# Glaciohound/Chimera-ST

Measured on AMD Instinct MI355X. Metric: train utterances/sec, MuST-C EN-DE s2t_transformer_m, 1/2/4/8 MI355X, higher is better.
Workload: dtype bf16

## Files before the change

chimera-st_amd/csrc/attention.hip:

```cpp
#include "cst_common.h"
#include <stdlib.h>
#include <type_traits>

namespace {

constexpr int NW = 4;
constexpr int QB = 32;
constexpr int KT = 64;

struct AttnParams {
  int64_t B, H, Tq, Tk;
  const void *Q, *K, *V; void* O;
  int64_t q_sb, q_sh, q_st, k_sb, k_sh, k_st, v_sb, v_sh, v_st, o_sb, o_sh, o_st;
  float* lse;
  const uint8_t* kpm; int64_t kpm_stride;
  int causal;
  float scale;
  const void* dO; int64_t do_sb, do_sh, do_st;
  void *dQ, *dK, *dV;
  int64_t dq_sb, dq_sh, dq_st, dk_sb, dk_sh, dk_st, dv_sb, dv_sh, dv_st;
  float* delta;
  uint32_t drop_thr, drop_key; float drop_scale;
  const int32_t* kv_len;
  uint8_t* q_flags;
  const int32_t* seq_off;
  const unsigned long long* kpm_bits; int64_t kpm_bits_stride;
};

struct SeqView { int64_t row0; int tq, tk; };
__device__ __forceinline__ SeqView seq_view(const AttnParams& p, int64_t b) {
  SeqView v;
  if (p.seq_off) {
    v.row0 = p.seq_off[b];
    v.tq = p.seq_off[b + 1] - p.seq_off[b];
    v.tk = p.kv_len ? (p.kv_len[b] < v.tq ? p.kv_len[b] : v.tq) : v.tq;
    if (v.tk < 0) v.tk = 0;
  } else {
    v.row0 = 0;
    v.tq = (int)p.Tq;
    v.tk = (int)p.Tk;
  }
  return v;
}

__device__ __forceinline__ int live_query_end(const AttnParams& p, int64_t b, int64_t h, int* sh, int tid, int tq) {
  const int nqt = (int)((p.Tq + 63) / 64);
  if (!p.q_flags) return tq;
  if (tid < 64) {
    const uint8_t* f = p.q_flags + (b * p.H + h) * nqt;
    int last = -1;
    for (int base = 0; base < nqt; base += 64) {
      const int idx = base + tid;
      const unsigned long long m = __ballot(idx < nqt && f[idx < nqt ? idx : 0] != 0);
      if (m) last = base + 63 - __clzll(m);
    }
    if (tid == 0) *sh = (last + 1) * 64;
  }
  __syncthreads();
  const int e = *sh;
  return e < tq ? e : tq;
}

__device__ __forceinline__ int slot_row(int t, int j, int hi) { return 16 * t + (j & 3) + 8 * (j >> 2) + 4 * hi; }

template <typename T, int D>
struct TileRegs {
  static constexpr int VEC = DT<T>::VEC, VPR = D / VEC, NV = (KT * VPR + NW * 64 - 1) / (NW * 64);
  u32x4 r[NV];
  __device__ __forceinline__ void fetch(const T* g, int64_t st, int nrows, int tid) {
#pragma unroll
    for (int i = 0; i < NV; ++i) {
      const int v = tid + NW * 64 * i;
      int row = v / VPR;
      row = row < nrows ? row : nrows - 1;
      if (v < KT * VPR) r[i] = *reinterpret_cast<const u32x4*>(g + (int64_t)row * st + (v % VPR) * VEC);
    }
  }
  __device__ __forceinline__ void stage(T* lds, int tid) const {
    constexpr int LD = D + VEC;
#pragma unroll
    for (int i = 0; i < NV; ++i) {
      const int v = tid + NW * 64 * i;
      if (v < KT * VPR) *reinterpret_cast<u32x4*>(lds + (v / VPR) * LD + (v % VPR) * VEC) = r[i];
    }
  }
};

template <typename T, int D>
__device__ __forceinline__ void load_row_frags(Frag<T> (&f)[D / 16], const T* g, int64_t st, int row, int nrows, int lane) {
  const int lk = 8 * (lane >> 5);
#pragma unroll
  for (int kk = 0; kk < D / 16; ++kk) {
    if (row < nrows) frag_load_contig(f[kk], g + (int64_t)row * st + kk * 16 + lk);
    else {
      float z[8] = {0, 0, 0, 0, 0, 0, 0, 0};
      frag_from_f32(f[kk], z);
    }
  }
}

template <typename T>
__device__ __forceinline__ void store_dcol(T* g, const f32x16& acc, int d0, int lane, float mul) {
  const int hi = lane >> 5;
#pragma unroll
  for (int gq = 0; gq < 4; ++gq) {
    T* p = g + d0 + 8 * gq + 4 * hi;
#pragma unroll
    for (int e = 0; e < 4; ++e) DT<T>::st(p + e, acc[gq * 4 + e] * mul);
  }
}

template <typename T, int D, bool DROP>
__global__ __launch_bounds__(NW * 64, (sizeof(T) == 2 ? 3 : 2)) void attn_fwd_kernel(AttnParams p) {
  constexpr int VEC = DT<T>::VEC, LD = D + VEC, TILE = KT * LD;
  extern __shared__ __attribute__((aligned(16))) char smem_raw[];
  T* smem = reinterpret_cast<T*>(smem_raw);
  unsigned long long* sMask = reinterpret_cast<unsigned long long*>(smem + 4 * TILE);
  const int tid = threadIdx.x, lane = tid & 63, wave = tid >> 6, hi = lane >> 5;
  const int64_t b = blockIdx.z, h = blockIdx.y;
  const int q_blk0 = blockIdx.x * (NW * QB);
  const int q = q_blk0 + wave * QB + (lane & 31);
  const SeqView sv = seq_view(p, b);
  if (q_blk0 >= sv.tq) return;
  const T* Qg = (const T*)p.Q + (p.seq_off ? sv.row0 * p.q_st : b * p.q_sb) + h * p.q_sh;
  const T* Kg = (const T*)p.K + (p.seq_off ? sv.row0 * p.k_st : b * p.k_sb) + h * p.k_sh;
  const T* Vg = (const T*)p.V + (p.seq_off ? sv.row0 * p.v_st : b * p.v_sb) + h * p.v_sh;
  const int cshift = sv.tk - sv.tq;
  const float c2 = p.scale * 1.4426950408889634f;
  const uint32_t dkey2 = cst_drop_key2(p.drop_key);
  const int thr_s = (int)p.drop_thr - 32768;
  const uint32_t rho = (uint32_t)((b * p.H + h) * p.Tq + q);
  cst_i32x4 bsig = {0, 0, 0, 0};
  if (DROP) bsig = cst_asig_row_frag(p.drop_key, dkey2, rho, hi);

  Frag<T> fq[D / 16];
  load_row_frags<T, D>(fq, Qg, p.q_st, q, sv.tq, lane);

  f32x16 o[D / 32];
#pragma unroll
  for (int dt = 0; dt < D / 32; ++dt)
#pragma unroll
    for (int r = 0; r < 16; ++r) o[dt][r] = 0.0f;
  float m_run = -1.0e30f, l_run = 0.0f;

  int64_t kend = sv.tk;
  if (!p.seq_off && p.kv_len && p.kv_len[b] < kend) kend = p.kv_len[b] > 0 ? p.kv_len[b] : 0;
  if (p.causal) {
    const int64_t last = (int64_t)q_blk0 + NW * QB - 1 + cshift + 1;
    if (last < kend) kend = last;
  }
  TileRegs<T, D> rk, rv;
  uint8_t rmask = 0;
  auto prefetch = [&](int64_t j0) {
    const int nk = (int)((sv.tk - j0 < KT) ? (sv.tk - j0) : KT);
    rk.fetch(Kg + j0 * p.k_st, p.k_st, nk, tid);
    rv.fetch(Vg + j0 * p.v_st, p.v_st, nk, tid);
    if (tid < KT) rmask = (tid >= nk) ? 1 : (p.kpm ? p.kpm[b * p.kpm_stride + j0 + tid] : 0);
  };
  auto stage = [&](int st) {
    rk.stage(smem + st * 2 * TILE, tid);
    rv.stage(smem + st * 2 * TILE + TILE, tid);
    if (wave == 0) {
      const unsigned long long bits = __ballot(rmask != 0);
      if (lane == 0) sMask[st] = bits;
    }
  };
  if (kend > 0) { prefetch(0); stage(0); }
  __syncthreads();
  int cur = 0;
  const int qlo = q_blk0 + wave * QB;
  for (int64_t j0 = 0; j0 < kend; j0 += KT) {
    const bool more = j0 + KT < kend;
    if (more) prefetch(j0 + KT);
    const T* sK = smem + cur * 2 * TILE;
    const T* sV = sK + TILE;
    const unsigned long long mb = sMask[cur];

    f32x16 s[2];
#pragma unroll
// ... 305 lines not shown

  f32x16 dk[D / 32], dv[D / 32];
#pragma unroll
  for (int dt = 0; dt < D / 32; ++dt)
#pragma unroll
    for (int r = 0; r < 16; ++r) { dk[dt][r] = 0.0f; dv[dt][r] = 0.0f; }

  int64_t qstart = 0;
  if (p.causal) {
    qstart = (int64_t)k_blk0 - cshift;
    if (qstart < 0) qstart = 0;
    qstart = (qstart / KT) * KT;
  }
  TileRegs<T, D> rq, rdo;
  float rl = -INFINITY, rd = 0.0f;
  auto prefetch = [&](int64_t i0) {
    const int nq = (int)((sv.tq - i0 < KT) ? (sv.tq - i0) : KT);
    rq.fetch(Qg + i0 * p.q_st, p.q_st, nq, tid);
    rdo.fetch(dOg + i0 * p.do_st, p.do_st, nq, tid);
    if (tid < KT) {
      const float l = tid < nq ? p.lse[(b * p.H + h) * p.Tq + i0 + tid] : -INFINITY;
      rl = l == -INFINITY ? INFINITY : l * 1.4426950408889634f;
      rd = tid < nq ? p.delta[(b * p.H + h) * p.Tq + i0 + tid] : 0.0f;
    }
  };
  auto stage = [&](int st) {
    rq.stage(smem + st * 2 * TILE, tid);
    rdo.stage(smem + st * 2 * TILE + TILE, tid);
    if (tid < KT) { sStat[st * 2 * KT + tid] = rl; sStat[st * 2 * KT + KT + tid] = rd; }
  };
  const int64_t qlim = live_query_end(p, b, h, reinterpret_cast<int*>(sStat + 4 * KT), tid, sv.tq);
  if (qstart < qlim) { prefetch(qstart); stage(0); }
  __syncthreads();
  int cur = 0;
  for (int64_t i0 = qstart; i0 < qlim; i0 += KT) {
    const bool more = i0 + KT < qlim;
    if (more) prefetch(i0 + KT);
    const T* sQ = smem + cur * 2 * TILE;
    const T* sdO = sQ + TILE;
    const float* sL = sStat + cur * 2 * KT;
    const float* sD = sL + KT;
#pragma unroll
    for (int qs = 0; qs < 2; ++qs) {
      f32x16 s, dp;
#pragma unroll
      for (int r = 0; r < 16; ++r) { s[r] = 0.0f; dp[r] = 0.0f; }
#pragma unroll
      for (int kk = 0; kk < D / 16; ++kk) {
        Frag<T> fqr, fdor;
        frag_load_contig(fqr, sQ + (qs * 32 + (lane & 31)) * LD + kk * 16 + 8 * hi);
        frag_load_contig(fdor, sdO + (qs * 32 + (lane & 31)) * LD + kk * 16 + 8 * hi);
        mma16(s, fqr, fk[kk]);
        mma16(dp, fdor, fv[kk]);
      }
      f32x16 pr;
      const bool diag = p.causal && (k_blk0 + wave * QB + QB - 1 > (int)i0 + qs * 32 + cshift);
      uint32_t keepbits = 0;
      if (DROP) {
        const cst_i32x16 dm = cst_asig_block(cst_asig_row_frag(p.drop_key, dkey2, rho0 + (uint32_t)((int)i0 + qs * 32 + (lane & 31)), hi), ksig);
#pragma unroll
        for (int r = 0; r < 16; ++r) keepbits |= (cst_adrop_keep(dm[r], thr_s) ? 1u : 0u) << r;
      }
#pragma unroll
      for (int r = 0; r < 16; ++r) {
        const int qr = qs * 32 + acc_row(r, lane);
        const float l = sL[qr];
        float e = __builtin_amdgcn_exp2f(fmaf(s[r], c2, -l));
        if (diag) e = (key > (int)i0 + qr + cshift) ? 0.0f : e;
        float dpr = dp[r];
        if (DROP) {
          const bool keep = (keepbits >> r) & 1u;
          dpr = keep ? dpr * p.drop_scale : 0.0f;
          pr[r] = keep ? e * p.drop_scale : 0.0f;
        } else {
          pr[r] = e;
        }
        s[r] = e * (dpr - sD[qr]);
      }
#pragma unroll
      for (int t = 0; t < 2; ++t) {
        Frag<T> fp, fds;
        float x[8], y[8];
#pragma unroll
        for (int j = 0; j < 8; ++j) { x[j] = pr[8 * t + j]; y[j] = s[8 * t + j]; }
        frag_from_f32(fp, x);
        frag_from_f32(fds, y);
#pragma unroll
        for (int dt = 0; dt < D / 32; ++dt) {
          Frag<T> fdot, fqt;
          frag_load_tr(fdot, sdO, LD, dt * 32, qs * 32 + 16 * t + 4 * hi, qs * 32 + 16 * t + 4 * hi + 8, lane);
          frag_load_tr(fqt, sQ, LD, dt * 32, qs * 32 + 16 * t + 4 * hi, qs * 32 + 16 * t + 4 * hi + 8, lane);
          mma16(dv[dt], fdot, fp);
          mma16(dk[dt], fqt, fds);
        }
      }
    }
    if (more) stage(cur ^ 1);
    __syncthreads();
    cur ^= 1;
  }
  if (key_masked) {
#pragma unroll
    for (int dt = 0; dt < D / 32; ++dt)
#pragma unroll
      for (int r = 0; r < 16; ++r) { dk[dt][r] = 0.0f; dv[dt][r] = 0.0f; }
  }
  if (key < krows) {
    T* gk = dKb + (int64_t)key * p.dk_st;
    T* gv = dVb + (int64_t)key * p.dv_st;
#pragma unroll
    for (int dt = 0; dt < D / 32; ++dt) {
      store_dcol<T>(gk, dk[dt], dt * 32, lane, p.scale);
      store_dcol<T>(gv, dv[dt], dt * 32, lane, 1.0f);
    }
  }
}

#include "attention_fast.inc"

int fill_params(const cst_attn_desc* d, AttnParams& p, bool bwd) {
  CST_REQUIRE(d, "cst_attn: null descriptor");
  CST_REQUIRE(d->dtype == CST_F32 || d->dtype == CST_BF16, "cst_attn: bad dtype %d", d->dtype);
  CST_REQUIRE(d->D == 32 || d->D == 64, "cst_attn: head dim %lld not in {32,64}", (long long)d->D);
  CST_REQUIRE(d->B > 0 && d->H > 0 && d->Tq > 0 && d->Tk > 0, "cst_attn: empty problem");
  CST_REQUIRE(d->Q && d->K && d->V && d->O && d->lse, "cst_attn: null tensor");
  CST_REQUIRE(d->H < 65536 && d->B < 65536, "cst_attn: B/H too large for the grid");
  const int vec = d->dtype == CST_BF16 ? 8 : 4;
  const int64_t strides[] = {d->q_sb, d->q_sh, d->q_st, d->k_sb, d->k_sh, d->k_st, d->v_sb, d->v_sh, d->v_st};
  for (int64_t s : strides) CST_REQUIRE(s % vec == 0, "cst_attn: strides must be multiples of %d elements", vec);
  CST_REQUIRE(((uintptr_t)d->Q % 16 == 0) && ((uintptr_t)d->K % 16 == 0) && ((uintptr_t)d->V % 16 == 0), "cst_attn: Q/K/V must be 16-byte aligned");
  p.B = d->B; p.H = d->H; p.Tq = d->Tq; p.Tk = d->Tk;
  p.Q = d->Q; p.K = d->K; p.V = d->V; p.O = d->O;
  p.q_sb = d->q_sb; p.q_sh = d->q_sh; p.q_st = d->q_st;
  p.k_sb = d->k_sb; p.k_sh = d->k_sh; p.k_st = d->k_st;
  p.v_sb = d->v_sb; p.v_sh = d->v_sh; p.v_st = d->v_st;
  p.o_sb = d->o_sb; p.o_sh = d->o_sh; p.o_st = d->o_st;
  p.lse = d->lse; p.kpm = d->key_padding_mask; p.kpm_stride = d->kpm_stride;
  p.causal = d->causal; p.scale = d->scale;
  CST_REQUIRE(d->drop_p >= 0.0f && d->drop_p < 1.0f, "cst_attn: drop_p must be in [0, 1)");
  CST_REQUIRE(d->drop_p == 0.0f || (double)d->B * d->H * d->Tq < 4294967296.0, "cst_attn: dropout row space exceeds 2^32 rows");
  p.drop_thr = d->drop_p > 0.0f ? cst_drop_thr16(d->drop_p) : 0u;
  p.drop_key = d->drop_key;
  p.drop_scale = d->drop_p > 0.0f ? 1.0f / (1.0f - d->drop_p) : 1.0f;
  p.dO = d->dO; p.do_sb = d->do_sb; p.do_sh = d->do_sh; p.do_st = d->do_st;
  p.dQ = d->dQ; p.dK = d->dK; p.dV = d->dV;
  p.dq_sb = d->dq_sb; p.dq_sh = d->dq_sh; p.dq_st = d->dq_st;
  p.dk_sb = d->dk_sb; p.dk_sh = d->dk_sh; p.dk_st = d->dk_st;
  p.dv_sb = d->dv_sb; p.dv_sh = d->dv_sh; p.dv_st = d->dv_st;
  p.delta = d->delta;
  p.kv_len = d->kv_len;
  p.seq_off = d->seq_offsets;
  p.kpm_bits = (const unsigned long long*)d->kpm_bits;
  p.kpm_bits_stride = (d->Tk + 63) / 64;
  if (p.seq_off) {
    CST_REQUIRE(d->Tq == d->Tk && d->key_padding_mask == nullptr, "cst_attn: packed sequences are self-attention (Tq == Tk = longest segment) without a key padding mask (kv_len gives the keys per sequence)");
    CST_REQUIRE(d->q_st == d->k_st && d->q_st == d->v_st, "cst_attn: packed Q/K/V must share one row stride");
  }
  p.q_flags = bwd ? d->q_flags : nullptr;
  if (bwd) {
    CST_REQUIRE(d->dO && d->dQ && d->dK && d->dV && d->delta, "cst_attn_bwd: null gradient tensor");
    CST_REQUIRE(d->do_sb % vec == 0 && d->do_sh % vec == 0 && d->do_st % vec == 0 && d->o_st % vec == 0 && d->o_sb % vec == 0 && d->o_sh % vec == 0,
                "cst_attn_bwd: dO/O strides must be multiples of %d", vec);
    CST_REQUIRE(((uintptr_t)d->dO % 16 == 0) && ((uintptr_t)d->O % 16 == 0), "cst_attn_bwd: dO/O must be 16-byte aligned");
  }
  return CST_OK;
}

template <typename T, int D>
constexpr size_t attn_lds_bytes() {
  return 4 * (size_t)KT * (D + DT<T>::VEC) * sizeof(T) + 4 * KT * sizeof(float) + 16;
}
void attn_set_lds(const void* fn) {
  (void)hipFuncSetAttribute(fn, hipFuncAttributeMaxDynamicSharedMemorySize, 96 * 1024);
}

double attn_flops(const cst_attn_desc* d, double gemms) {
  double pairs = (double)d->Tq * (double)d->Tk;
  if (d->causal) pairs *= 0.5;
  return gemms * 2.0 * pairs * (double)d->D * (double)d->B * (double)d->H;
}

bool attn_fast_ok(const cst_attn_desc* d) {
  const bool off = getenv("CST_ATTN_GENERIC") != nullptr;
  return !off && d->dtype == CST_BF16 && d->D == 64 && !d->causal && (d->key_padding_mask == nullptr || d->kpm_bits != nullptr) &&
         d->Tk <= 65536 && (int64_t)d->Tk * d->k_st < (1ll << 29) && (int64_t)d->Tq * d->q_st < (1ll << 29) && (int64_t)d->Tk * d->v_st < (1ll << 29) &&
         d->o_st % 8 == 0 && d->o_sh % 8 == 0 && d->o_sb % 8 == 0 && (uintptr_t)d->O % 16 == 0;
}
bool attn_fast_bwd_ok(const cst_attn_desc* d) {
  const int64_t st[] = {d->dq_sb, d->dq_sh, d->dq_st, d->dk_sb, d->dk_sh, d->dk_st, d->dv_sb, d->dv_sh, d->dv_st};
  for (int64_t x : st) if (x % 8) return false;
  return attn_fast_ok(d) && d->bwd_ws != nullptr && (uintptr_t)d->dQ % 16 == 0 && (uintptr_t)d->dK % 16 == 0 && (uintptr_t)d->dV % 16 == 0 &&
         (uintptr_t)d->bwd_ws % 16 == 0 && (int64_t)d->Tq * d->do_st < (1ll << 29);
}

}

extern "C" int cst_attn_fwd(const cst_attn_desc* d, cst_stream stream) {
  AttnParams p;
  int rc = fill_params(d, p, false);
  if (rc != CST_OK) return rc;
  hipStream_t s = (hipStream_t)stream;
  if (attn_fast_ok(d)) {
    CstProfScope prof(CST_K_ATTN_FWD, s, attn_flops(d, 2.0), 0.0);
    const unsigned nblk = fa_grid(d->Tq, d->B, d->H);
    const size_t lds = FA_NSLOT * FA_SLOT + 8 * (size_t)cst_ceil_div(d->Tk, 64) + (p.drop_thr ? 4096 : 0);
    if (p.drop_thr) hipLaunchKernelGGL((fa_fwd_kernel<true>), dim3(nblk), dim3(256), lds, s, p);
    else hipLaunchKernelGGL((fa_fwd_kernel<false>), dim3(nblk), dim3(256), lds, s, p);
    return cst_check_launch("cst_attn_fwd");
  }
  dim3 grid((unsigned)cst_ceil_div(d->Tq, NW * QB), (unsigned)d->H, (unsigned)d->B);
  CstProfScope prof(CST_K_ATTN_FWD, s, attn_flops(d, 2.0), 0.0);
#define CST_FWD1(T, DD, DR) do { const size_t lds = attn_lds_bytes<T, DD>(); attn_set_lds(reinterpret_cast<const void*>(&attn_fwd_kernel<T, DD, DR>)); \
    hipLaunchKernelGGL((attn_fwd_kernel<T, DD, DR>), grid, dim3(NW * 64), lds, s, p); } while (0)
#define CST_FWD(T, DD) do { if (p.drop_thr) CST_FWD1(T, DD, true); else CST_FWD1(T, DD, false); } while (0)
  if (d->dtype == CST_BF16) { if (d->D == 64) CST_FWD(bf16_t, 64); else CST_FWD(bf16_t, 32); }
  else { if (d->D == 64) CST_FWD(float, 64); else CST_FWD(float, 32); }
#undef CST_FWD
#undef CST_FWD1
  return cst_check_launch("cst_attn_fwd");
}

int cst_fa_dec_cross(const void* q, const void* kx, const void* vx, const uint8_t* kpm, void* out, const int32_t* step, int64_t max_len,
                     int64_t bsz, int64_t beam, int64_t H, int64_t S, float scale, const void* Wg, const float* sg, const float* sb, float eps,
                     int64_t K, int64_t ldx, hipStream_t s) {
  if (Wg) {
    FdProj pj = {(const bf16_t*)Wg, sg, sb, eps, (int)K, (long long)ldx};
    return fa_dec_cross_launch(q, kx, vx, kpm, out, step, max_len, bsz, beam, H, S, scale, &pj, s);
  }
  return fa_dec_cross_launch(q, kx, vx, kpm, out, step, max_len, bsz, beam, H, S, scale, nullptr, s);
}

extern "C" int64_t cst_attn_bwd_workspace(const cst_attn_desc* d) {
  if (!d) return 0;
  return (int64_t)d->B * d->H * cst_ceil_div(d->Tq, 64) * 64 * (int64_t)(2 * sizeof(float) + 32);
}

extern "C" int cst_attn_bwd(const cst_attn_desc* d, cst_stream stream) {
  AttnParams p;
  int rc = fill_params(d, p, true);
  if (rc != CST_OK) return rc;
  hipStream_t s = (hipStream_t)stream;
  CstProfScope prof(CST_K_ATTN_BWD, s, attn_flops(d, 5.0), 0.0);
  if (attn_fast_bwd_ok(d)) {
    const int64_t Tq64 = cst_ceil_div(d->Tq, 64) * 64;
    float* ws = (float*)d->bwd_ws;
    static const bool delta_pass = getenv("CST_ATTN_DELTA_PASS") != nullptr;
    if (delta_pass) hipLaunchKernelGGL(fa_delta_kernel, dim3((unsigned)(Tq64 / 64), (unsigned)d->H, (unsigned)d->B), dim3(64), 0, s, p, ws, Tq64);
    const unsigned nq = fa_grid(d->Tq, d->B, d->H), nk = fa_grid(d->Tk, d->B, d->H);
    const size_t lds_q = FA_NSLOT * FA_SLOT + 8 * (size_t)cst_ceil_div(d->Tk, 64) + (p.drop_thr ? 4096 : 0) + 16, lds_k = FA_NSLOT * (FA_SLOT + FA_STATS);
    if (p.drop_thr) {
      hipLaunchKernelGGL((fa_dq_kernel<true>), dim3(nq), dim3(256), lds_q, s, p, ws, Tq64);
      hipLaunchKernelGGL((fa_dkv_kernel<true>), dim3(nk), dim3(256), lds_k, s, p, (const float*)ws, Tq64);
    } else {
      hipLaunchKernelGGL((fa_dq_kernel<false>), dim3(nq), dim3(256), lds_q, s, p, ws, Tq64);
      hipLaunchKernelGGL((fa_dkv_kernel<false>), dim3(nk), dim3(256), lds_k, s, p, (const float*)ws, Tq64);
    }
    return cst_check_launch("cst_attn_bwd");
  }
  dim3 gq((unsigned)cst_ceil_div(d->Tq, NW * QB), (unsigned)d->H, (unsigned)d->B);
  dim3 gk((unsigned)cst_ceil_div(d->Tk, NW * QB), (unsigned)d->H, (unsigned)d->B);
#define CST_BWD1(T, DD, DR)                                                                                \
  do {                                                                                                     \
    hipLaunchKernelGGL((attn_delta_kernel<T, DD>), dim3((unsigned)cst_ceil_div(d->Tq, 64), (unsigned)d->H, (unsigned)d->B), dim3(64), 0, s, p); \
    const size_t lds = attn_lds_bytes<T, DD>();                                                              \
    attn_set_lds(reinterpret_cast<const void*>(&attn_bwd_dq_kernel<T, DD, DR>));                             \
    attn_set_lds(reinterpret_cast<const void*>(&attn_bwd_dkv_kernel<T, DD, DR>));                            \
    hipLaunchKernelGGL((attn_bwd_dq_kernel<T, DD, DR>), gq, dim3(NW * 64), lds, s, p);                      \
    hipLaunchKernelGGL((attn_bwd_dkv_kernel<T, DD, DR>), gk, dim3(NW * 64), lds, s, p);                     \
  } while (0)
#define CST_BWD(T, DD) do { if (p.drop_thr) CST_BWD1(T, DD, true); else CST_BWD1(T, DD, false); } while (0)
  if (d->dtype == CST_BF16) { if (d->D == 64) CST_BWD(bf16_t, 64); else CST_BWD(bf16_t, 32); }
  else { if (d->D == 64) CST_BWD(float, 64); else CST_BWD(float, 32); }
#undef CST_BWD
#undef CST_BWD1
  return cst_check_launch("cst_attn_bwd");
}
```

chimera-st_amd/csrc/attention_fast.inc:

```

typedef int fa_i32x4 __attribute__((ext_vector_type(4)));
constexpr int FA_IMG = 64 * 128;
constexpr int FA_SLOT = 2 * FA_IMG;
constexpr int FA_NSLOT = 3;
constexpr float FA_THR = 8.0f;

__device__ __forceinline__ int fa_sw(int r) {
  const int s = (r >> 1) & 7;
  return s ^ ((s & 1) << 2);
}
__device__ __forceinline__ fa_i32x4 fa_rsrc(const void* base, uint32_t bytes) {
  const unsigned long long a = (unsigned long long)base;
  fa_i32x4 r;
  r[0] = __builtin_amdgcn_readfirstlane((int)(unsigned)a);
  r[1] = __builtin_amdgcn_readfirstlane((int)(unsigned)(a >> 32));
  r[2] = __builtin_amdgcn_readfirstlane((int)bytes);
  r[3] = 0x00020000;
  return r;
}
__device__ __forceinline__ void fa_dma16(const fa_i32x4& rs, unsigned lds, unsigned voff) {
  unsigned keep;
  asm volatile("s_mov_b32 %0, m0\n\ts_mov_b32 m0, %1\n\ts_nop 0\n\tbuffer_load_dwordx4 %2, %3, 0 offen lds\n\ts_mov_b32 m0, %0"
               : "=&s"(keep) : "s"(lds), "v"(voff), "s"(rs) : "memory");
}
__device__ __forceinline__ void fa_dma4(const fa_i32x4& rs, unsigned lds, unsigned voff) {
  unsigned keep;
  asm volatile("s_mov_b32 %0, m0\n\ts_mov_b32 m0, %1\n\ts_nop 0\n\tbuffer_load_dword %2, %3, 0 offen lds\n\ts_mov_b32 m0, %0"
               : "=&s"(keep) : "s"(lds), "v"(voff), "s"(rs) : "memory");
}
__device__ __forceinline__ void fa_dma_tile4(const fa_i32x4& rsA, const fa_i32x4& rsB, unsigned lds, unsigned a0, unsigned a1, unsigned b0, unsigned b1) {
  unsigned keep;
  asm volatile("s_mov_b32 %0, m0\n\ts_mov_b32 m0, %1\n\ts_nop 0\n\tbuffer_load_dwordx4 %2, %6, 0 offen lds\n\t"
               "s_add_i32 m0, %1, 0x400\n\ts_nop 0\n\tbuffer_load_dwordx4 %3, %6, 0 offen lds\n\t"
               "s_add_i32 m0, %1, 0x2000\n\ts_nop 0\n\tbuffer_load_dwordx4 %4, %7, 0 offen lds\n\t"
               "s_add_i32 m0, %1, 0x2400\n\ts_nop 0\n\tbuffer_load_dwordx4 %5, %7, 0 offen lds\n\ts_mov_b32 m0, %0"
               : "=&s"(keep) : "s"(lds), "v"(a0), "v"(a1), "v"(b0), "v"(b1), "s"(rsA), "s"(rsB) : "memory");
}
template <int N> __device__ __forceinline__ void fa_wait_vm() { asm volatile("s_waitcnt vmcnt(%0)" ::"n"(N) : "memory"); }

__device__ __forceinline__ void fa_dma_lanes(unsigned (&v)[2], int64_t st, int wave, int lane) {
#pragma unroll
  for (int i = 0; i < 2; ++i) {
    const int row = 8 * (2 * wave + i) + (lane >> 3);
    v[i] = (unsigned)(row * (int)st * 2 + ((((lane & 7) ^ fa_sw(row))) << 4));
  }
}
struct FaLanes {
  unsigned row[4];
  unsigned ta[2];
  unsigned tb[2];
};
__device__ __forceinline__ FaLanes fa_lanes(int lane) {
  FaLanes L;
  const int hi = lane >> 5, lrow = lane & 31, swl = fa_sw(lrow);
#pragma unroll
  for (int kk = 0; kk < 4; ++kk) L.row[kk] = (unsigned)(lrow * 128 + (((2 * kk + hi) ^ swl) << 4));
  const int s = lane & 15, r0 = 4 * hi + (s >> 2), cc = 2 * ((lane >> 4) & 1) + ((s & 3) >> 1), cb = 8 * (s & 1);
#pragma unroll
  for (int dt = 0; dt < 2; ++dt) {
    L.ta[dt] = (unsigned)(r0 * 128 + (((4 * dt + cc) ^ fa_sw(r0)) << 4) + cb);
    L.tb[dt] = (unsigned)((r0 + 8) * 128 + (((4 * dt + cc) ^ fa_sw(r0 + 8)) << 4) + cb);
  }
  return L;
}
__device__ __forceinline__ bf16x8 fa_ld_row(const char* img, unsigned off) { return *reinterpret_cast<const bf16x8*>(img + off); }
__device__ __forceinline__ bf16x8 fa_ld_tr(const char* img, unsigned oa, unsigned ob) {
  const v4s_t x = __builtin_amdgcn_ds_read_tr16_b64_v4i16((v4s_t __attribute__((address_space(3)))*)(img + oa));
  const v4s_t y = __builtin_amdgcn_ds_read_tr16_b64_v4i16((v4s_t __attribute__((address_space(3)))*)(img + ob));
  u16x8 t;
  t[0] = (unsigned short)x[0]; t[1] = (unsigned short)x[1]; t[2] = (unsigned short)x[2]; t[3] = (unsigned short)x[3];
  t[4] = (unsigned short)y[0]; t[5] = (unsigned short)y[1]; t[6] = (unsigned short)y[2]; t[7] = (unsigned short)y[3];
  return __builtin_bit_cast(bf16x8, t);
}
typedef short fa_s16x2 __attribute__((ext_vector_type(2)));
typedef float fa_f32x2 __attribute__((ext_vector_type(2)));
typedef __bf16 fa_bf16x2 __attribute__((ext_vector_type(2)));
__device__ __forceinline__ unsigned fa_pack2(float lo, float hi) {
  const fa_f32x2 v = {lo, hi};
  return __builtin_bit_cast(unsigned, __builtin_convertvector(v, fa_bf16x2));
}
__device__ __forceinline__ fa_s16x2 fa_thrm1(uint32_t thr16) {
  const short t = (short)((int)thr16 - 32768 - 1);
  fa_s16x2 v = {t, t};
  return v;
}
__device__ __forceinline__ unsigned fa_keep_pair(unsigned packed, int d0, int d1, fa_s16x2 thrm1) {
  fa_s16x2 h = __builtin_bit_cast(fa_s16x2, __builtin_amdgcn_perm((unsigned)d1, (unsigned)d0, 0x05040100u));
  h = h << 2;
  fa_s16x2 t = __builtin_elementwise_sub_sat(thrm1, h);
  t = t >> 15;
  return packed & __builtin_bit_cast(unsigned, t);
}
template <bool KEYS>
__device__ __forceinline__ void fa_stage_sigs(char* dst, uint32_t key, uint32_t key2, uint32_t row0, int tid) {
  const uint32_t r = row0 + (uint32_t)(tid >> 2);
  const int w = 2 * (tid & 3);
  uint2 v;
  v.x = KEYS ? cst_asig_key(key, key2, r, w) : cst_asig_row(key, key2, r, w);
  v.y = KEYS ? cst_asig_key(key, key2, r, w + 1) : cst_asig_row(key, key2, r, w + 1);
  *reinterpret_cast<uint2*>(dst + (tid >> 2) * 32 + (tid & 3) * 8) = v;
}
__device__ __forceinline__ cst_i32x16 fa_mask_block(const char* sigs, int blk, int lane, const cst_i32x4& own) {
  const cst_i32x4 a = *reinterpret_cast<const cst_i32x4*>(sigs + (blk * 32 + (lane & 31)) * 32 + 16 * (lane >> 5));
  return cst_asig_block(a, own);
}
#define FA_MFMA(a, b, c) __builtin_amdgcn_mfma_f32_32x32x16_bf16(a, b, c, 0, 0, 0)

__device__ __forceinline__ float fa_other_half(float x) {
  const unsigned u = __float_as_uint(x);
  const auto r = __builtin_amdgcn_permlane32_swap(u, u, false, false);
  return __uint_as_float((threadIdx.x & 32) ? r[0] : r[1]);
}
__device__ __forceinline__ void fa_row_frags(bf16x8 (&f)[4], const bf16_t* g, int64_t st, int row, int nrows, int hi, float mul) {
  const int rc = row < nrows ? row : nrows - 1;
  const float m = row < nrows ? mul : 0.0f;
  u32x4 raw[4];
#pragma unroll
  for (int kk = 0; kk < 4; ++kk) raw[kk] = *reinterpret_cast<const u32x4*>(g + (int64_t)rc * st + kk * 16 + 8 * hi);
#pragma unroll
  for (int kk = 0; kk < 4; ++kk) {
    u32x4 w;
#pragma unroll
    for (int i = 0; i < 4; ++i) w[i] = fa_pack2(__uint_as_float(raw[kk][i] << 16) * m, __uint_as_float(raw[kk][i] & 0xffff0000u) * m);
    f[kk] = __builtin_bit_cast(bf16x8, w);
  }
}
template <typename T> __device__ __forceinline__ const T* fa_uniform(const T* p) {
  const unsigned long long a = (unsigned long long)p;
  const unsigned lo = (unsigned)__builtin_amdgcn_readfirstlane((int)(unsigned)a), hi = (unsigned)__builtin_amdgcn_readfirstlane((int)(unsigned)(a >> 32));
  return (const T*)(((unsigned long long)hi << 32) | lo);
}
__device__ __forceinline__ unsigned long long fa_tile_bits(const unsigned long long* kb_lds, int j, int kend) {
  if (kb_lds) {
    const unsigned long long v = kb_lds[j];
    const unsigned lo = (unsigned)__builtin_amdgcn_readfirstlane((int)(unsigned)v), hi = (unsigned)__builtin_amdgcn_readfirstlane((int)(unsigned)(v >> 32));
    return ((unsigned long long)hi << 32) | lo;
  }
  const int left = kend - 64 * j;
  return left >= 64 ? 0ull : (~0ull << left);
}
__device__ __forceinline__ void fa_store_row(bf16_t* rowp, const f32x16 (&acc)[2], float mul, int hi) {
#pragma unroll
  for (int dt = 0; dt < 2; ++dt)
#pragma unroll
    for (int gp = 0; gp < 2; ++gp) {
      unsigned a[2], c[2];
#pragma unroll
      for (int e = 0; e < 2; ++e) {
        a[e] = fa_pack2(acc[dt][8 * gp + 2 * e] * mul, acc[dt][8 * gp + 2 * e + 1] * mul);
        c[e] = fa_pack2(acc[dt][8 * gp + 4 + 2 * e] * mul, acc[dt][8 * gp + 4 + 2 * e + 1] * mul);
      }
      const auto r0 = __builtin_amdgcn_permlane32_swap(a[0], c[0], false, false);
      const auto r1 = __builtin_amdgcn_permlane32_swap(a[1], c[1], false, false);
      u32x4 v = {r0[0], r1[0], r0[1], r1[1]};
      *reinterpret_cast<u32x4*>(rowp + dt * 32 + 16 * gp + 8 * hi) = v;
    }
}

__device__ __forceinline__ bool fa_block_coords(const AttnParams& p, int nxb, int& xb, int64_t& h, int64_t& b) {
  const unsigned id = blockIdx.x, xcd = id & 7, k = id >> 3;
  const unsigned g = (k / (unsigned)nxb) * 8 + xcd;
  xb = __builtin_amdgcn_readfirstlane((int)(k % (unsigned)nxb));
  h = __builtin_amdgcn_readfirstlane((int)(g % (unsigned)p.H));
  b = __builtin_amdgcn_readfirstlane((int)(g / (unsigned)p.H));
  return g < (unsigned)(p.B * p.H);
}
inline unsigned fa_grid(int64_t rows, int64_t B, int64_t H) { return (unsigned)(8 * cst_ceil_div(rows, 128) * cst_ceil_div(B * H, 8)); }

#ifdef CST_TRACE
#define FA_STAMP(i) do { if (tr && tid == 0) { tr[2 * (i)] = (long long)__builtin_readcyclecounter(); tr[2 * (i) + 1] = (long long)__builtin_amdgcn_s_memrealtime(); } } while (0)
#else
#define FA_STAMP(i) do { } while (0)
#endif

template <bool DROP>
__global__ __launch_bounds__(256, 3) void fa_fwd_kernel(AttnParams p) {
  extern __shared__ __attribute__((aligned(16))) char smem_raw[];
  const int tid = threadIdx.x, lane = tid & 63, hi = lane >> 5;
  const int wave = __builtin_amdgcn_readfirstlane(tid >> 6);
#ifdef CST_TRACE
  long long* tr = p.delta ? reinterpret_cast<long long*>(p.delta) + (size_t)blockIdx.x * 16 : nullptr;
#endif
  FA_STAMP(0);
  int xb; int64_t b, h;
  if (!fa_block_coords(p, (int)((p.Tq + 127) / 128), xb, h, b)) return;
  const int q_blk0 = xb * 128;
  const SeqView sv = seq_view(p, b);
  if (q_blk0 >= sv.tq) return;
  const int q = q_blk0 + wave * 32 + (lane & 31);
  const bf16_t* Qg = (const bf16_t*)p.Q + (p.seq_off ? sv.row0 * p.q_st : b * p.q_sb) + h * p.q_sh;
  const bf16_t* Kg = (const bf16_t*)p.K + (p.seq_off ? sv.row0 * p.k_st : b * p.k_sb) + h * p.k_sh;
  const bf16_t* Vg = (const bf16_t*)p.V + (p.seq_off ? sv.row0 * p.v_st : b * p.v_sb) + h * p.v_sh;
  int kend = sv.tk;
  if (!p.seq_off && p.kv_len && p.kv_len[b] < kend) kend = p.kv_len[b] > 0 ? p.kv_len[b] : 0;
  const int ntiles = (kend + 63) >> 6;
  const int ntmax = (int)((p.Tk + 63) >> 6);
  unsigned long long* kbits = p.kpm_bits ? reinterpret_cast<unsigned long long*>(smem_raw + FA_NSLOT * FA_SLOT) : nullptr;
  char* const sigs = smem_raw + FA_NSLOT * FA_SLOT + 8 * ntmax;
  const unsigned lds0 = (unsigned)(uintptr_t)(__attribute__((address_space(3))) char*)smem_raw;
  const fa_i32x4 rsK = fa_rsrc(Kg, kend > 0 ? (uint32_t)((kend - 1) * p.k_st * 2 + 128) : 0u);
  const fa_i32x4 rsV = fa_rsrc(Vg, kend > 0 ? (uint32_t)((kend - 1) * p.v_st * 2 + 128) : 0u);
  unsigned vk[2], vv[2];
  fa_dma_lanes(vk, p.k_st, wave, lane);
  fa_dma_lanes(vv, p.v_st, wave, lane);
  const unsigned stepK = (unsigned)(64 * p.k_st * 2), stepV = (unsigned)(64 * p.v_st * 2);
  auto dma_tile = [&](int j, int slot) {
    fa_dma_tile4(rsK, rsV, lds0 + slot * FA_SLOT + wave * 2048, vk[0] + (unsigned)j * stepK, vk[1] + (unsigned)j * stepK,
                 vv[0] + (unsigned)j * stepV, vv[1] + (unsigned)j * stepV);
  };
  if (ntiles > 0) dma_tile(0, 0);
  if (ntiles > 1) dma_tile(1, 1);

  const float c2 = p.scale * 1.4426950408889634f;
  bf16x8 fq[4];
  fa_row_frags(fq, Qg, p.q_st, q, sv.tq, hi, c2);
  const uint32_t dkey2 = cst_drop_key2(p.drop_key);
  cst_i32x4 bsig = {0, 0, 0, 0};
  if (DROP) {
    bsig = cst_asig_row_frag(p.drop_key, dkey2, (uint32_t)((b * p.H + h) * p.Tq + q), hi);
    fa_stage_sigs<true>(sigs, p.drop_key, dkey2, 0u, tid);
  }
  if (kbits) for (int j = tid; j < ntiles; j += 256) kbits[j] = p.kpm_bits[b * p.kpm_bits_stride + j];
  const FaLanes L = fa_lanes(lane);
  const fa_s16x2 thrm1 = fa_thrm1(p.drop_thr);

  f32x16 o[2], negm;
#pragma unroll
  for (int r = 0; r < 16; ++r) { o[0][r] = 0.0f; o[1][r] = 0.0f; negm[r] = 0.0f; }
  float l_run = 0.0f, raise_at = -INFINITY;

  FA_STAMP(1);
  fa_wait_vm<0>();
  __syncthreads();
  FA_STAMP(2);

  auto tile = [&](int j, auto slot_c) {
    constexpr int SLOT = decltype(slot_c)::value;
    const bool ahead = j + 2 < ntiles;
    if (ahead) dma_tile(j + 2, (SLOT + 2) % FA_NSLOT);
    const char* sK = smem_raw + SLOT * FA_SLOT;
    const char* sV = sK + FA_IMG;
    const unsigned long long mb = fa_tile_bits(kbits, j, kend);
    f32x16 s[2];
    if (__builtin_expect(mb != 0ull, 0)) {
      const unsigned long long mbl = mb >> (4 * hi);
#pragma unroll
      for (int ks = 0; ks < 2; ++ks) {
        f32x16 cm;
#pragma unroll
        for (int r = 0; r < 16; ++r) cm[r] = ((mbl >> (ks * 32 + (r & 3) + 8 * (r >> 2))) & 1ull) ? -INFINITY : negm[r];
        s[ks] = FA_MFMA(fa_ld_row(sK, L.row[0] + ks * 4096), fq[0], cm);
#pragma unroll
        for (int kk = 1; kk < 4; ++kk) s[ks] = FA_MFMA(fa_ld_row(sK, L.row[kk] + ks * 4096), fq[kk], s[ks]);
      }
    } else {
#pragma unroll
      for (int ks = 0; ks < 2; ++ks) {
        s[ks] = FA_MFMA(fa_ld_row(sK, L.row[0] + ks * 4096), fq[0], negm);
#pragma unroll
        for (int kk = 1; kk < 4; ++kk) s[ks] = FA_MFMA(fa_ld_row(sK, L.row[kk] + ks * 4096), fq[kk], s[ks]);
      }
    }
    float mt = s[0][0];
#pragma unroll
    for (int ks = 0; ks < 2; ++ks)
#pragma unroll
      for (int r = 0; r < 16; ++r) mt = fmaxf(mt, s[ks][r]);
    mt = fmaxf(mt, fa_other_half(mt));
    if (__builtin_expect(__any(mt > raise_at), 0)) {
      const bool need = mt > raise_at;
      const bool first = raise_at < 0.0f;
      const float dm = need ? ceilf(mt) : 0.0f;
      const float alpha = first ? 1.0f : __builtin_amdgcn_exp2f(-dm);
#pragma unroll
      for (int r = 0; r < 16; ++r) { o[0][r] *= alpha; o[1][r] *= alpha; negm[r] -= dm; s[0][r] -= dm; s[1][r] -= dm; }
      l_run *= alpha;
      raise_at = need ? FA_THR : raise_at;
    }
    fa_f32x2 l01 = {0.0f, 0.0f};
#pragma unroll
    for (int ks = 0; ks < 2; ++ks)
#pragma unroll
      for (int r = 0; r < 16; r += 2) {
        s[ks][r] = __builtin_amdgcn_exp2f(s[ks][r]);
        s[ks][r + 1] = __builtin_amdgcn_exp2f(s[ks][r + 1]);
        const fa_f32x2 pr = {s[ks][r], s[ks][r + 1]};
        l01 = l01 + pr;
      }
    l_run += l01[0] + l01[1];
    unsigned pk[2][8];
#pragma unroll
    for (int ks = 0; ks < 2; ++ks)
#pragma unroll
      for (int i = 0; i < 8; ++i) pk[ks][i] = fa_pack2(s[ks][2 * i], s[ks][2 * i + 1]);
    if (DROP) {
      if (j + 1 < ntiles) fa_stage_sigs<true>(sigs + ((j + 1) & 1) * 2048, p.drop_key, dkey2, (uint32_t)(64 * (j + 1)), tid);
#pragma unroll
      for (int ks = 0; ks < 2; ++ks) {
        const cst_i32x16 dm = fa_mask_block(sigs + (j & 1) * 2048, ks, lane, bsig);
#pragma unroll
        for (int i = 0; i < 8; ++i) pk[ks][i] = fa_keep_pair(pk[ks][i], dm[2 * i], dm[2 * i + 1], thrm1);
      }
    }
#pragma unroll
    for (int ks = 0; ks < 2; ++ks)
#pragma unroll
      for (int t = 0; t < 2; ++t) {
        const u32x4 fpw = {pk[ks][4 * t], pk[ks][4 * t + 1], pk[ks][4 * t + 2], pk[ks][4 * t + 3]};
        const bf16x8 fp = __builtin_bit_cast(bf16x8, fpw);
#pragma unroll
        for (int dt = 0; dt < 2; ++dt)
          o[dt] = FA_MFMA(fa_ld_tr(sV, L.ta[dt] + ks * 4096 + t * 2048, L.tb[dt] + ks * 4096 + t * 2048), fp, o[dt]);
      }
    if (ahead) fa_wait_vm<4>(); else fa_wait_vm<0>();
    if (DROP) __syncthreads();
    else __builtin_amdgcn_s_barrier();
  };
  for (int j = 0; j < ntiles; j += 3) {
    tile(j, std::integral_constant<int, 0>{});
    if (j + 1 < ntiles) tile(j + 1, std::integral_constant<int, 1>{});
    if (j + 2 < ntiles) tile(j + 2, std::integral_constant<int, 2>{});
  }
  FA_STAMP(3);
  const float l_tot = l_run + fa_other_half(l_run);
  if (q < sv.tq) {
    const float inv = l_tot > 0.0f ? p.drop_scale / l_tot : 0.0f;
    bf16_t* Og = (bf16_t*)p.O + (p.seq_off ? sv.row0 * p.o_st : b * p.o_sb) + h * p.o_sh + (int64_t)q * p.o_st;
    fa_store_row(Og, o, inv, hi);
    if (hi == 0) p.lse[(b * p.H + h) * p.Tq + q] = l_tot > 0.0f ? (__log2f(l_tot) - negm[0]) * 0.6931471805599453f : -INFINITY;
  }
#ifdef CST_TRACE
  FA_STAMP(4);
  if (tr && tid == 0) { tr[10] = (long long)__builtin_amdgcn_s_getreg(4 | (0 << 6) | (31 << 11)); tr[11] = ntiles; }
#endif
}

__global__ __launch_bounds__(64) void fa_delta_kernel(AttnParams p, float* ws, int64_t Tq64) {
  const int64_t b = blockIdx.z, h = blockIdx.y;
  const int qt = blockIdx.x, lane = threadIdx.x;
  const int rl = lane >> 3, c8 = (lane & 7) * 8;
  bool nz = false;
  const SeqView sv = seq_view(p, b);
  const bf16_t* obase = (const bf16_t*)p.O + (p.seq_off ? sv.row0 * p.o_st : b * p.o_sb) + h * p.o_sh + c8;
  const bf16_t* gbase = (const bf16_t*)p.dO + (p.seq_off ? sv.row0 * p.do_st : b * p.do_sb) + h * p.do_sh + c8;
  float* w0 = ws + ((b * p.H + h) * 2) * Tq64;
  const float inv_ds = 1.0f / p.drop_scale;
#pragma unroll
  for (int it = 0; it < 8; ++it) {
    const int64_t q = (int64_t)qt * 64 + it * 8 + rl;
    float acc = 0.0f;
    if (q < sv.tq) {
      float a[8], c[8];
      load8(obase + q * p.o_st, a);
      load8(gbase + q * p.do_st, c);
#pragma unroll
      for (int e = 0; e < 8; ++e) { acc += a[e] * c[e]; nz = nz || c[e] != 0.0f; }
    }
    acc += __shfl_xor(acc, 1, 64);
    acc += __shfl_xor(acc, 2, 64);
    acc += __shfl_xor(acc, 4, 64);
    if ((lane & 7) == 0) {
      float nl = -INFINITY;
      if (q < sv.tq) {
        const float l = p.lse[(b * p.H + h) * p.Tq + q];
        nl = l == -INFINITY ? -INFINITY : -l * 1.4426950408889634f;
      }
      w0[q] = nl;
      w0[Tq64 + q] = q < sv.tq ? -acc * inv_ds : 0.0f;
    }
  }
  const unsigned long long m = __ballot(nz);
  if (p.q_flags && lane == 0) p.q_flags[(b * p.H + h) * ((p.Tq + 63) / 64) + qt] = m != 0ull ? 1 : 0;
}

__device__ __forceinline__ f32x16 fa_masked_c(const f32x16& c, unsigned long long mbl, int ks) {
  f32x16 cm;
#pragma unroll
  for (int r = 0; r < 16; ++r) cm[r] = ((mbl >> (ks * 32 + (r & 3) + 8 * (r >> 2))) & 1ull) ? -INFINITY : c[r];
  return cm;
}

template <bool DROP>
__global__ __launch_bounds__(256, 2) void fa_dq_kernel(AttnParams p, float* ws, int64_t Tq64) {
  extern __shared__ __attribute__((aligned(16))) char smem_raw[];
  const int tid = threadIdx.x, lane = tid & 63, hi = lane >> 5;
  const int wave = __builtin_amdgcn_readfirstlane(tid >> 6);
  int xb; int64_t b, h;
  if (!fa_block_coords(p, (int)((p.Tq + 127) / 128), xb, h, b)) return;
  const int q_blk0 = xb * 128;
  const SeqView sv = seq_view(p, b);
  const int nqt = (int)((p.Tq + 63) / 64);
  uint8_t* const qfl = p.q_flags ? p.q_flags + (b * p.H + h) * nqt + 2 * xb : nullptr;
  if (q_blk0 >= sv.tq) {
    if (qfl && tid < 2 && 2 * xb + tid < nqt) qfl[tid] = 0;
    return;
  }
  const int q = q_blk0 + wave * 32 + (lane & 31);
  const bf16_t* Qg = (const bf16_t*)p.Q + (p.seq_off ? sv.row0 * p.q_st : b * p.q_sb) + h * p.q_sh;
  const bf16_t* Kg = (const bf16_t*)p.K + (p.seq_off ? sv.row0 * p.k_st : b * p.k_sb) + h * p.k_sh;
  const bf16_t* Vg = (const bf16_t*)p.V + (p.seq_off ? sv.row0 * p.v_st : b * p.v_sb) + h * p.v_sh;
  const bf16_t* dOg = (const bf16_t*)p.dO + (p.seq_off ? sv.row0 * p.do_st : b * p.do_sb) + h * p.do_sh;
  const bf16_t* Og = (const bf16_t*)p.O + (p.seq_off ? sv.row0 * p.o_st : b * p.o_sb) + h * p.o_sh;
  bf16_t* const dQb = (bf16_t*)p.dQ + (p.seq_off ? sv.row0 * p.dq_st : b * p.dq_sb) + h * p.dq_sh;
  int kend = sv.tk;
  if (!p.seq_off && p.kv_len && p.kv_len[b] < kend) kend = p.kv_len[b] > 0 ? p.kv_len[b] : 0;
  const int ntiles = (kend + 63) >> 6;
  const int ntmax = (int)((p.Tk + 63) >> 6);
  unsigned long long* kbits = p.kpm_bits ? reinterpret_cast<unsigned long long*>(smem_raw + FA_NSLOT * FA_SLOT) : nullptr;
  char* const sigs = smem_raw + FA_NSLOT * FA_SLOT + 8 * ntmax;
  int* const sh_nz = reinterpret_cast<int*>(smem_raw + FA_NSLOT * FA_SLOT + 8 * ntmax + (DROP ? 4096 : 0));
  const unsigned lds0 = (unsigned)(uintptr_t)(__attribute__((address_space(3))) char*)smem_raw;
  const fa_i32x4 rsK = fa_rsrc(Kg, kend > 0 ? (uint32_t)((kend - 1) * p.k_st * 2 + 128) : 0u);
  const fa_i32x4 rsV = fa_rsrc(Vg, kend > 0 ? (uint32_t)((kend - 1) * p.v_st * 2 + 128) : 0u);
  unsigned vk[2], vv[2];
  fa_dma_lanes(vk, p.k_st, wave, lane);
  fa_dma_lanes(vv, p.v_st, wave, lane);
  const unsigned stepK = (unsigned)(64 * p.k_st * 2), stepV = (unsigned)(64 * p.v_st * 2);
  auto dma_tile = [&](int j, int slot) {
    fa_dma_tile4(rsK, rsV, lds0 + slot * FA_SLOT + wave * 2048, vk[0] + (unsigned)j * stepK, vk[1] + (unsigned)j * stepK,
                 vv[0] + (unsigned)j * stepV, vv[1] + (unsigned)j * stepV);
  };
  if (ntiles > 0) dma_tile(0, 0);
  if (ntiles > 1) dma_tile(1, 1);

  const float c2 = p.scale * 1.4426950408889634f;
  bf16x8 fq[4], fdo[4];
  fa_row_frags(fq, Qg, p.q_st, q, sv.tq, hi, c2);
  fa_row_frags(fdo, dOg, p.do_st, q, sv.tq, hi, 1.0f);
  float ndv, nl = -INFINITY;
  bool nzrow = false;
  {
    float acc = 0.0f;
    const int rc = q < sv.tq ? q : sv.tq - 1;
#pragma unroll
    for (int kk = 0; kk < 4; ++kk) {
      const u32x4 ro = *reinterpret_cast<const u32x4*>(Og + (int64_t)rc * p.o_st + kk * 16 + 8 * hi);
      const u32x4 rg = __builtin_bit_cast(u32x4, fdo[kk]);
#pragma unroll
      for (int i = 0; i < 4; ++i) {
        acc += __uint_as_float(ro[i] << 16) * __uint_as_float(rg[i] << 16);
        acc += __uint_as_float(ro[i] & 0xffff0000u) * __uint_as_float(rg[i] & 0xffff0000u);
        nzrow = nzrow || (rg[i] & 0x7fff7fffu) != 0u;
      }
    }
    acc += __shfl_xor(acc, 32, 64);
    if (q < sv.tq) {
      const float l = p.lse[(b * p.H + h) * p.Tq + q];
      nl = l == -INFINITY ? -INFINITY : -l * 1.4426950408889634f;
    }
    ndv = q < sv.tq ? -acc * (1.0f / p.drop_scale) : 0.0f;
    if (hi == 0 && q < Tq64) {
      float* w0 = ws + ((b * p.H + h) * 2) * Tq64;
      w0[q] = nl;
      w0[Tq64 + q] = ndv;
    }
    const unsigned long long m = __ballot(nzrow);
    if (lane == 0) sh_nz[wave] = m != 0ull ? 1 : 0;
  }
  f32x16 nl2, nd, dq[2];
#pragma unroll
  for (int r = 0; r < 16; ++r) { nl2[r] = nl; nd[r] = ndv; dq[0][r] = 0.0f; dq[1][r] = 0.0f; }
  const uint32_t dkey2 = cst_drop_key2(p.drop_key);
  const int thr_s = (int)p.drop_thr - 32768;
  cst_i32x4 bsig = {0, 0, 0, 0};
  if (DROP) {
    bsig = cst_asig_row_frag(p.drop_key, dkey2, (uint32_t)((b * p.H + h) * p.Tq + q), hi);
    fa_stage_sigs<true>(sigs, p.drop_key, dkey2, 0u, tid);
    if (q < Tq64) {
      cst_i32x4* sg = reinterpret_cast<cst_i32x4*>(reinterpret_cast<char*>(ws + (size_t)p.B * p.H * 2 * Tq64) + ((size_t)(b * p.H + h) * Tq64 + q) * 32 + 16 * hi);
      *sg = bsig;
    }
  }
  if (kbits) for (int j = tid; j < ntiles; j += 256) kbits[j] = p.kpm_bits[b * p.kpm_bits_stride + j];
  const FaLanes L = fa_lanes(lane);
  fa_wait_vm<0>();
  __syncthreads();
  {
    const int nz01 = sh_nz[0] | sh_nz[1], nz23 = sh_nz[2] | sh_nz[3];
    if (qfl && tid == 0) {
      qfl[0] = (uint8_t)nz01;
      if (2 * xb + 1 < nqt) qfl[1] = (uint8_t)nz23;
    }
    if (!(nz01 | nz23)) {
      if (q < sv.tq) {
        f32x16 z[2];
#pragma unroll
        for (int r = 0; r < 16; ++r) { z[0][r] = 0.0f; z[1][r] = 0.0f; }
        fa_store_row(dQb + (int64_t)q * p.dq_st, z, 1.0f, hi);
      }
      return;
    }
  }

  auto tile = [&](int j, auto slot_c) {
    constexpr int SLOT = decltype(slot_c)::value;
    const bool ahead = j + 2 < ntiles;
    if (ahead) dma_tile(j + 2, (SLOT + 2) % FA_NSLOT);
    const char* sK = smem_raw + SLOT * FA_SLOT;
    const char* sV = sK + FA_IMG;
    const unsigned long long mb = fa_tile_bits(kbits, j, kend);
    const unsigned long long mbl = mb >> (4 * hi);
    if (DROP && j + 1 < ntiles) fa_stage_sigs<true>(sigs + ((j + 1) & 1) * 2048, p.drop_key, dkey2, (uint32_t)(64 * (j + 1)), tid);
#pragma unroll
    for (int ks = 0; ks < 2; ++ks) {
      f32x16 s, dp;
      if (__builtin_expect(mb != 0ull, 0)) s = FA_MFMA(fa_ld_row(sK, L.row[0] + ks * 4096), fq[0], fa_masked_c(nl2, mbl, ks));
      else s = FA_MFMA(fa_ld_row(sK, L.row[0] + ks * 4096), fq[0], nl2);
      dp = FA_MFMA(fa_ld_row(sV, L.row[0] + ks * 4096), fdo[0], nd);
#pragma unroll
      for (int kk = 1; kk < 4; ++kk) {
        s = FA_MFMA(fa_ld_row(sK, L.row[kk] + ks * 4096), fq[kk], s);
        dp = FA_MFMA(fa_ld_row(sV, L.row[kk] + ks * 4096), fdo[kk], dp);
      }
      if (DROP) {
        const cst_i32x16 dm = fa_mask_block(sigs + (j & 1) * 2048, ks, lane, bsig);
#pragma unroll
        for (int r = 0; r < 16; ++r) dp[r] = cst_adrop_keep(dm[r], thr_s) ? dp[r] : ndv;
      }
#pragma unroll
      for (int r = 0; r < 16; ++r) s[r] = __builtin_amdgcn_exp2f(s[r]) * dp[r];
#pragma unroll
      for (int t = 0; t < 2; ++t) {
        const u32x4 fw = {fa_pack2(s[8 * t], s[8 * t + 1]), fa_pack2(s[8 * t + 2], s[8 * t + 3]), fa_pack2(s[8 * t + 4], s[8 * t + 5]), fa_pack2(s[8 * t + 6], s[8 * t + 7])};
        const bf16x8 fds = __builtin_bit_cast(bf16x8, fw);
#pragma unroll
        for (int dt = 0; dt < 2; ++dt)
          dq[dt] = FA_MFMA(fa_ld_tr(sK, L.ta[dt] + ks * 4096 + t * 2048, L.tb[dt] + ks * 4096 + t * 2048), fds, dq[dt]);
      }
    }
    if (ahead) fa_wait_vm<4>(); else fa_wait_vm<0>();
    if (DROP) __syncthreads();
    else __builtin_amdgcn_s_barrier();
  };
  for (int j = 0; j < ntiles; j += 3) {
    tile(j, std::integral_constant<int, 0>{});
    if (j + 1 < ntiles) tile(j + 1, std::integral_constant<int, 1>{});
    if (j + 2 < ntiles) tile(j + 2, std::integral_constant<int, 2>{});
  }
  if (q < sv.tq) fa_store_row(dQb + (int64_t)q * p.dq_st, dq, p.scale * p.drop_scale, hi);
}

constexpr int FA_STATS = 2 * 256 + 2048;

template <bool DROP>
__global__ __launch_bounds__(256, 2) void fa_dkv_kernel(AttnParams p, const float* ws, int64_t Tq64) {
  extern __shared__ __attribute__((aligned(16))) char smem_raw[];
  constexpr int SLOTB = FA_SLOT + FA_STATS;
  const int tid = threadIdx.x, lane = tid & 63, hi = lane >> 5;
  const int wave = __builtin_amdgcn_readfirstlane(tid >> 6);
  int xb; int64_t b, h;
  if (!fa_block_coords(p, (int)((p.Tk + 127) / 128), xb, h, b)) return;
  const int k_blk0 = xb * 128;
  const SeqView sv = seq_view(p, b);
  const int krows = p.seq_off ? sv.tq : sv.tk;
  if (k_blk0 >= krows) return;
  const int key = k_blk0 + wave * 32 + (lane & 31);
  const bf16_t* Qg = (const bf16_t*)p.Q + (p.seq_off ? sv.row0 * p.q_st : b * p.q_sb) + h * p.q_sh;
  const bf16_t* Kg = (const bf16_t*)p.K + (p.seq_off ? sv.row0 * p.k_st : b * p.k_sb) + h * p.k_sh;
  const bf16_t* Vg = (const bf16_t*)p.V + (p.seq_off ? sv.row0 * p.v_st : b * p.v_sb) + h * p.v_sh;
  const bf16_t* dOg = (const bf16_t*)p.dO + (p.seq_off ? sv.row0 * p.do_st : b * p.do_sb) + h * p.do_sh;
  bf16_t* const dKb = (bf16_t*)p.dK + (p.seq_off ? sv.row0 * p.dk_st : b * p.dk_sb) + h * p.dk_sh;
  bf16_t* const dVb = (bf16_t*)p.dV + (p.seq_off ? sv.row0 * p.dv_st : b * p.dv_sb) + h * p.dv_sh;
  int kend = sv.tk;
  if (!p.seq_off && p.kv_len && p.kv_len[b] < kend) kend = p.kv_len[b] > 0 ? p.kv_len[b] : 0;
  const int qlim = live_query_end(p, b, h, reinterpret_cast<int*>(smem_raw), tid, sv.tq);
  if (k_blk0 >= kend || qlim <= 0) {
    if (key < krows) {
      f32x16 z[2];
#pragma unroll
      for (int r = 0; r < 16; ++r) { z[0][r] = 0.0f; z[1][r] = 0.0f; }
      fa_store_row(dKb + (int64_t)key * p.dk_st, z, 1.0f, hi);
      fa_store_row(dVb + (int64_t)key * p.dv_st, z, 1.0f, hi);
    }
    return;
  }
  __syncthreads();
  const int ntiles = (qlim + 63) >> 6;
  const unsigned lds0 = (unsigned)(uintptr_t)(__attribute__((address_space(3))) char*)smem_raw;
  const fa_i32x4 rsQ = fa_rsrc(Qg, (uint32_t)((sv.tq - 1) * p.q_st * 2 + 128));
  const fa_i32x4 rsO = fa_rsrc(dOg, (uint32_t)((sv.tq - 1) * p.do_st * 2 + 128));
  const float* w0 = ws + ((b * p.H + h) * 2) * Tq64;
  const fa_i32x4 rsS = fa_rsrc(w0, (uint32_t)(2 * Tq64 * 4));
  const fa_i32x4 rsG = fa_rsrc(reinterpret_cast<const char*>(ws + (size_t)p.B * p.H * 2 * Tq64) + (size_t)(b * p.H + h) * Tq64 * 32, (uint32_t)(Tq64 * 32));
  unsigned vq[2], vo[2];
  fa_dma_lanes(vq, p.q_st, wave, lane);
  fa_dma_lanes(vo, p.do_st, wave, lane);
  const unsigned stepQ = (unsigned)(64 * p.q_st * 2), stepO = (unsigned)(64 * p.do_st * 2);
  const uint32_t dkey2 = cst_drop_key2(p.drop_key);
  const int thr_s = (int)p.drop_thr - 32768;
  auto dma_tile = [&](int j, int slot) {
    fa_dma_tile4(rsQ, rsO, lds0 + slot * SLOTB + wave * 2048, vq[0] + (unsigned)j * stepQ, vq[1] + (unsigned)j * stepQ,
                 vo[0] + (unsigned)j * stepO, vo[1] + (unsigned)j * stepO);
    if (wave < 2) fa_dma4(rsS, lds0 + slot * SLOTB + FA_SLOT + wave * 256, (unsigned)((j * 64 + lane) * 4) + (unsigned)wave * (unsigned)(Tq64 * 4));
    else if (DROP) fa_dma16(rsG, lds0 + slot * SLOTB + FA_SLOT + 512 + (wave - 2) * 1024, (unsigned)(j * 2048 + (wave - 2) * 1024 + lane * 16));
  };
  dma_tile(0, 0);
  if (ntiles > 1) dma_tile(1, 1);

  const float c2 = p.scale * 1.4426950408889634f;
  bf16x8 fk[4], fv[4];
  fa_row_frags(fk, Kg, p.k_st, key, kend, hi, c2);
  fa_row_frags(fv, Vg, p.v_st, key, kend, hi, 1.0f);
  bool key_masked = key >= kend;
  if (p.kpm_bits && key < kend) key_masked = (p.kpm_bits[b * p.kpm_bits_stride + (key >> 6)] >> (key & 63)) & 1ull;
  cst_i32x4 ksig = {0, 0, 0, 0};
  if (DROP) ksig = cst_asig_key_frag(p.drop_key, dkey2, (uint32_t)key, hi);
  f32x16 dk[2], dv[2];
#pragma unroll
  for (int r = 0; r < 16; ++r) { dk[0][r] = 0.0f; dk[1][r] = 0.0f; dv[0][r] = 0.0f; dv[1][r] = 0.0f; }
  const FaLanes L = fa_lanes(lane);
  const unsigned srow = (unsigned)(16 * hi);
  fa_wait_vm<0>();
  __syncthreads();

  auto tile = [&](int j, auto slot_c) {
    constexpr int SLOT = decltype(slot_c)::value;
    const bool ahead = j + 2 < ntiles;
    if (ahead) dma_tile(j + 2, (SLOT + 2) % FA_NSLOT);
    const char* sQ = smem_raw + SLOT * SLOTB;
    const char* sdO = sQ + FA_IMG;
    const char* sS = sQ + FA_SLOT + srow;
#pragma unroll
    for (int qs = 0; qs < 2; ++qs) {
      f32x16 s, dp, nd;
#pragma unroll
      for (int g = 0; g < 4; ++g) {
        const f32x4 a = *reinterpret_cast<const f32x4*>(sS + (qs * 32 + 8 * g) * 4);
        const f32x4 c = *reinterpret_cast<const f32x4*>(sS + 256 + (qs * 32 + 8 * g) * 4);
#pragma unroll
        for (int e = 0; e < 4; ++e) { s[4 * g + e] = a[e]; nd[4 * g + e] = c[e]; }
      }
      dp = FA_MFMA(fa_ld_row(sdO, L.row[0] + qs * 4096), fv[0], nd);
      s = FA_MFMA(fa_ld_row(sQ, L.row[0] + qs * 4096), fk[0], s);
#pragma unroll
      for (int kk = 1; kk < 4; ++kk) {
        s = FA_MFMA(fa_ld_row(sQ, L.row[kk] + qs * 4096), fk[kk], s);
        dp = FA_MFMA(fa_ld_row(sdO, L.row[kk] + qs * 4096), fv[kk], dp);
      }
      f32x16 pr;
#pragma unroll
      for (int r = 0; r < 16; ++r) pr[r] = __builtin_amdgcn_exp2f(s[r]);
      if (DROP) {
        const cst_i32x16 dm = fa_mask_block(sQ + FA_SLOT + 512, qs, lane, ksig);
#pragma unroll
        for (int r = 0; r < 16; ++r) {
          const bool keep = cst_adrop_keep(dm[r], thr_s);
          s[r] = pr[r] * (keep ? dp[r] : nd[r]);
          pr[r] = keep ? pr[r] : 0.0f;
        }
      } else {
#pragma unroll
        for (int r = 0; r < 16; ++r) s[r] = pr[r] * dp[r];
      }
#pragma unroll
      for (int t = 0; t < 2; ++t) {
        const u32x4 pw = {fa_pack2(pr[8 * t], pr[8 * t + 1]), fa_pack2(pr[8 * t + 2], pr[8 * t + 3]), fa_pack2(pr[8 * t + 4], pr[8 * t + 5]), fa_pack2(pr[8 * t + 6], pr[8 * t + 7])};
        const u32x4 dw = {fa_pack2(s[8 * t], s[8 * t + 1]), fa_pack2(s[8 * t + 2], s[8 * t + 3]), fa_pack2(s[8 * t + 4], s[8 * t + 5]), fa_pack2(s[8 * t + 6], s[8 * t + 7])};
        const bf16x8 fp = __builtin_bit_cast(bf16x8, pw), fds = __builtin_bit_cast(bf16x8, dw);
#pragma unroll
        for (int dt = 0; dt < 2; ++dt) {
          dv[dt] = FA_MFMA(fa_ld_tr(sdO, L.ta[dt] + qs * 4096 + t * 2048, L.tb[dt] + qs * 4096 + t * 2048), fp, dv[dt]);
          dk[dt] = FA_MFMA(fa_ld_tr(sQ, L.ta[dt] + qs * 4096 + t * 2048, L.tb[dt] + qs * 4096 + t * 2048), fds, dk[dt]);
        }
      }
    }
    if (!ahead) fa_wait_vm<0>();
    else if (DROP || wave < 2) fa_wait_vm<5>();
    else fa_wait_vm<4>();
    __syncthreads();
  };
  for (int j = 0; j < ntiles; j += 3) {
    tile(j, std::integral_constant<int, 0>{});
    if (j + 1 < ntiles) tile(j + 1, std::integral_constant<int, 1>{});
    if (j + 2 < ntiles) tile(j + 2, std::integral_constant<int, 2>{});
  }
  if (key_masked) {
#pragma unroll
    for (int r = 0; r < 16; ++r) { dk[0][r] = 0.0f; dk[1][r] = 0.0f; dv[0][r] = 0.0f; dv[1][r] = 0.0f; }
  }
  if (key < krows) {
    fa_store_row(dKb + (int64_t)key * p.dk_st, dk, p.scale * p.drop_scale, hi);
    fa_store_row(dVb + (int64_t)key * p.dv_st, dv, p.drop_scale, hi);
  }
}
// ... 255 lines not shown
```

chimera-st_amd/functional.py:

```python
import os as _os
import weakref as _weakref

import torch

from . import kernels as K
from . import lib as L

_ACT = {None: L.ACT_NONE, "none": L.ACT_NONE, "relu": L.ACT_RELU, "gelu": L.ACT_GELU}


def _flat2d(x):
    return x.reshape(-1, x.shape[-1]).contiguous()


def _vec(dtype):
    return 8 if dtype == torch.bfloat16 else 4


def _with_tiles(t, tiles):
    if t.is_contiguous():
        t._cst_live_tiles = (tiles[0], tiles[1], t.data_ptr(), t.numel(), t.shape[-1], t._version)
        if t._base is not None:
            t._base._cst_live_tiles = t._cst_live_tiles
    return t
# ... 269 lines not shown
        ctx.bias_objs = (b1, b2)
        return y.view(*x.shape[:-1], dout)

    @staticmethod
    def backward(ctx, dy):
        x2, w1, w2, z1, h = ctx.saved_tensors
        act, has_b1, has_b2, has_res, xshape = ctx.cfg
        M, d = x2.shape
        F_, dout = w1.shape[0], w2.shape[0]
        dy2 = _flat2d(dy)
        live = _tiles_of(dy, M)
        p_act, key_act, p_out, key_out = ctx.drop
        b1, b2 = ctx.bias_objs
        db2_fused = None
        gcs = not _os.environ.get("CST_NO_GEMM_COLSUM")
        db2_in_dw = gcs and has_b2 and ctx.needs_input_grad[4] and ctx.needs_input_grad[3] and dout % 8 == 0 and K.dw_colsum_is_fused(dout, F_, M, w2.dtype)
        db1_in_dw = gcs and has_b1 and ctx.needs_input_grad[2] and ctx.needs_input_grad[1] and F_ % 8 == 0 and K.dw_colsum_is_fused(F_, d, M, w1.dtype)
        if p_out > 0.0:
            dy2, db2_fused = _drop_grad(dy2, (p_out, key_out), w2.dtype, live, defer=_may_defer(w2, b2),
                                        with_colsum=not db2_in_dw and has_b2 and ctx.needs_input_grad[4] and dout % 8 == 0)
        use_wt = _want_wt(M, w2) and _want_wt(M, w1)
        dz1 = _dx_gemm(dy2, w2, M, use_wt=use_wt, like=dy2, dact=act, aux_in=z1, drop=(p_act, key_act), m_live=live)
        dx = dw1 = db1 = dw2 = db2 = None
        if ctx.needs_input_grad[3]:
            dw2, db2 = _dw_gemm(dy2, h, w2, b2, M, db_in_dw=db2_in_dw, live=live, dz_travels_on=dy2.data_ptr() == dy.data_ptr() and has_res)
        if has_b2 and ctx.needs_input_grad[4] and db2 is None:
            db2 = db2_fused if db2_fused is not None else K.colsum(dy2, w2.dtype, live, defer=_may_defer(w2, b2))
        if ctx.needs_input_grad[0]:
            dx = _dx_gemm(dz1, w1, M, use_wt=use_wt, like=x2, resid=_flat2d(dy) if ctx.res_is_x else None, m_live=live).view(xshape)
        if ctx.needs_input_grad[1]:
            dw1, db1 = _dw_gemm(dz1, x2, w1, b1, M, db_in_dw=db1_in_dw, live=live, dz_travels_on=False)
        if has_b1 and ctx.needs_input_grad[2] and db1 is None:
            db1 = K.colsum(dz1, w1.dtype, live, defer=_may_defer(w1, b1))
        dres = dy if has_res and ctx.needs_input_grad[5] and not (ctx.res_is_x and ctx.needs_input_grad[0]) else None
        return dx, dw1, db1, dw2, db2, dres, None, None, None, None, None


def ffn(x, w1, b1, w2, b2, act, resid=None, activation_dropout_p=0.0, dropout_p=0.0):
    assert _ACT[act] != L.ACT_NONE
    return _FFNFn.apply(x, w1.contiguous(), b1, w2.contiguous(), b2, resid, _ACT[act], *_drop_args(activation_dropout_p), *_drop_args(dropout_p))


class _LayerNormFn(torch.autograd.Function):
    @staticmethod
    def forward(ctx, x, res, gamma, beta, eps):
        x2 = _flat2d(x)
        r2 = _flat2d(res) if res is not None else None
        y, s, mean, rstd = K.layernorm_fwd(x2, r2, gamma, beta, eps, want_sum=True)
        src = s if res is not None else x2
        ctx.save_for_backward(src, gamma, mean, rstd)
        ctx.has_res = res is not None
        ctx.shape = x.shape
        ctx.set_materialize_grads(False)
        if res is not None:
            return y.view(x.shape), s.view(x.shape)
        return y.view(x.shape), None

    @staticmethod
    def backward(ctx, dy, ds):
        src, gamma, mean, rstd = ctx.saved_tensors
        if dy is None:
            return ds, (ds if ctx.has_res else None), None, None, None
        dy2 = _flat2d(dy)
        dres = _flat2d(ds) if ds is not None else None
        dx, dg, db, tiles = K.layernorm_bwd(dy2, src, gamma, mean, rstd, dres, grad_dtype=gamma.dtype, want_tiles=True, defer=_may_defer(gamma))
        dx = _with_tiles(dx.view(ctx.shape), tiles)
        return dx, (dx if ctx.has_res else None), dg, db, None


def layer_norm(x, gamma, beta, eps=1e-5):
    return _LayerNormFn.apply(x, None, gamma, beta, eps)[0]


def add_layer_norm(x, res, gamma, beta, eps=1e-5):
    return _LayerNormFn.apply(x, res, gamma, beta, eps)


class _LayerNormPassFn(torch.autograd.Function):

    @staticmethod
    def forward(ctx, x, gamma, beta, eps):
        x2 = _flat2d(x)
        y, _, mean, rstd = K.layernorm_fwd(x2, None, gamma, beta, eps)
        ctx.save_for_backward(x2, gamma, mean, rstd)
        ctx.shape = x.shape
        ctx.set_materialize_grads(False)
        return y.view(x.shape), x.view_as(x)

    @staticmethod
    def backward(ctx, dy, dxp):
        x2, gamma, mean, rstd = ctx.saved_tensors
        dres = _flat2d(dxp) if dxp is not None else None
        if dy is None:
            return (dxp, None, None, None)
        dx, dg, db = K.layernorm_bwd(_flat2d(dy), x2, gamma, mean, rstd, dres, grad_dtype=gamma.dtype, defer=_may_defer(gamma))
        return dx.view(ctx.shape), dg, db, None


def layer_norm_residual(x, gamma, beta, eps=1e-5):
    return _LayerNormPassFn.apply(x, gamma, beta, eps)


_MASK_CACHE = []


_PAD_TILES = []


def _pad_tiles(u8):
    for src, pt in _PAD_TILES:
        if src is u8:
            return pt
    flat = u8.reshape(-1)
    pad = (-flat.numel()) % 64
    if pad:
        flat = torch.cat([flat, torch.ones(pad, dtype=flat.dtype, device=flat.device)])
    pt = flat.view(-1, 64).amin(dim=1) > 0
    _PAD_TILES.append((u8, pt))
    if len(_PAD_TILES) > 8:
        _PAD_TILES.pop(0)
    return pt


def _mask_and_len(key_padding_mask):
    if key_padding_mask is None:
        return None, None
    if _os.environ.get("CST_ATTN_NO_KVLEN"):
        return key_padding_mask.to(torch.uint8).contiguous(), None
    for src, ver, u8, kvl in _MASK_CACHE:
        if src is key_padding_mask and ver == key_padding_mask._version:
            return u8, kvl
    u8 = key_padding_mask.to(torch.uint8).contiguous()
    Tk = u8.shape[1]
    pos = torch.arange(1, Tk + 1, device=u8.device, dtype=torch.int32)
    kvl = (pos * (u8 == 0)).amax(dim=1).to(torch.int32).contiguous()
    _MASK_CACHE.append((key_padding_mask, key_padding_mask._version, u8, kvl))
    if len(_MASK_CACHE) > 8:
        _MASK_CACHE.pop(0)
    return u8, kvl


def _laid_out_like(do, o):
    if do.stride() == o.stride():
        return do
    tmp = torch.empty_like(o)
    tmp.copy_(do)
    return tmp


class _AttnFn(torch.autograd.Function):
    @staticmethod
    def forward(ctx, q, k, v, kpm, kvl, H, causal, scale, layout_q, layout_kv, drop_p, drop_key):
        D = q.shape[-1] // H
        o, lse = K.attn_fwd(q, k, v, H, D, kpm, causal, scale, layout_q, layout_kv, drop_p, drop_key, kvl)
        ctx.save_for_backward(q, k, v, o, lse, kpm, kvl)
        ctx.cfg = (H, D, causal, scale, layout_q, layout_kv, drop_p, drop_key)
        return o

    @staticmethod
    def backward(ctx, do):
        q, k, v, o, lse, kpm, kvl = ctx.saved_tensors
        H, D, causal, scale, lq, lkv, drop_p, drop_key = ctx.cfg
        dq, dk, dv = K.attn_bwd(_laid_out_like(do, o), q, k, v, o, lse, H, D, kpm, causal, scale, lq, lkv, drop_p, drop_key, kvl)
        return dq, dk, dv, None, None, None, None, None, None, None, None, None


class _AttnKVFn(torch.autograd.Function):

    @staticmethod
    def forward(ctx, q, kv, kpm, kvl, H, scale, drop_p, drop_key):
        C = kv.shape[-1] // 2
        D = C // H
        k, v = kv[..., :C], kv[..., C:]
        o, lse = K.attn_fwd(q, k, v, H, D, kpm, False, scale, "bt", "bt", drop_p, drop_key, kvl)
        ctx.save_for_backward(q, kv, o, lse, kpm, kvl)
        ctx.cfg = (H, D, C, scale, drop_p, drop_key)
        return o

    @staticmethod
    def backward(ctx, do):
        q, kv, o, lse, kpm, kvl = ctx.saved_tensors
        H, D, C, scale, drop_p, drop_key = ctx.cfg
        dq, dkv = torch.empty_like(q), torch.empty_like(kv)
        K.attn_bwd(_laid_out_like(do, o), q, kv[..., :C], kv[..., C:], o, lse, H, D, kpm, False, scale, "bt", "bt", drop_p, drop_key, kvl,
                   grads=(dq, dkv[..., :C], dkv[..., C:]))
        return dq, dkv, None, None, None, None, None, None


def attention_kv(q, kv, num_heads, key_padding_mask=None, scale=None, dropout_p=0.0):
    C = q.shape[-1]
    if scale is None:
        scale = (C // num_heads) ** -0.5
    key_padding_mask, kv_len = _mask_and_len(key_padding_mask)
    assert q.stride(-1) == 1 and kv.is_contiguous() and kv.shape[-1] == 2 * C
    return _AttnKVFn.apply(q, kv, key_padding_mask, kv_len, num_heads, float(scale), *_drop_args(dropout_p))


def _drop_args(dropout_p):
    if dropout_p and dropout_p > 0.0:
        from . import rng
        return float(dropout_p), rng.next_key()
    return 0.0, 0


def attention(q, k, v, num_heads, key_padding_mask=None, causal=False, scale=None, layout_q="bt", layout_kv="bt", dropout_p=0.0):
    if scale is None:
        scale = (q.shape[-1] // num_heads) ** -0.5
    key_padding_mask, kv_len = _mask_and_len(key_padding_mask)
    assert q.stride(-1) == 1 and k.stride(-1) == 1 and v.stride(-1) == 1
    return _AttnFn.apply(q, k, v, key_padding_mask, kv_len, num_heads, bool(causal), float(scale), layout_q, layout_kv,
                         *_drop_args(dropout_p))


def attention_avg_probs(q, k, num_heads, key_padding_mask=None, scale=None):
    if torch.is_grad_enabled() and (q.requires_grad or k.requires_grad):
        raise NotImplementedError("attention weights are computed under torch.no_grad() only")
    if scale is None:
        scale = (q.shape[-1] // num_heads) ** -0.5
    if key_padding_mask is not None and key_padding_mask.dim() == 0:
        key_padding_mask = None
    return K.attn_avg_probs(q, k, num_heads, key_padding_mask, float(scale))


class _AttnPackedFn(torch.autograd.Function):

    @staticmethod
    def forward(ctx, qkv, kpm, kvl, H, causal, scale, drop_p, drop_key, pad_tiles=None, seq=None):
        ctx.pad_tiles = pad_tiles
        C = qkv.shape[-1] // 3
        D = C // H
        q, k, v = qkv[..., :C], qkv[..., C:2 * C], qkv[..., 2 * C:]
        B, T = qkv.shape[0], qkv.shape[1]
        o = torch.empty(B, T, C, dtype=qkv.dtype, device=qkv.device)
        lse = torch.empty((seq[0].numel() - 1) if seq is not None else B, H, int(seq[1]) if seq is not None else T, dtype=torch.float32, device=qkv.device)
        d = K.attn_desc(q, k, v, o, lse, H, D, kpm, causal, scale, "bt", "bt", drop_p, drop_key, kvl, seq)
        K.attn_fwd_desc(d)
        ctx.save_for_backward(qkv, o, lse, kpm, kvl, seq[0] if seq is not None else None)
        ctx.cfg = (H, D, C, causal, scale, drop_p, drop_key, int(seq[1]) if seq is not None else None)
        return o

    @staticmethod
    def backward(ctx, do):
        qkv, o, lse, kpm, kvl, seq_off = ctx.saved_tensors
        H, D, C, causal, scale, drop_p, drop_key, seq_max = ctx.cfg
        seq = (seq_off, seq_max) if seq_off is not None else None
        live = _tiles_of(do, qkv.shape[0] * qkv.shape[1]) if ctx.pad_tiles is not None else None
        if not do.is_contiguous():
            do = do.contiguous()
        dqkv = torch.empty_like(qkv)
        K.attn_bwd(do, qkv[..., :C], qkv[..., C:2 * C], qkv[..., 2 * C:], o, lse, H, D, kpm, causal, scale, "bt", "bt", drop_p, drop_key, kvl, seq,
                   grads=(dqkv[..., :C], dqkv[..., C:2 * C], dqkv[..., 2 * C:]))
        if live is not None:
            stamps = torch.where(ctx.pad_tiles, live[0], torch.full_like(live[0], live[1] if live[1] < 2 ** 31 else live[1] - 2 ** 32))
            dqkv = _with_tiles(dqkv, (stamps, live[1]))
        return dqkv, None, None, None, None, None, None, None, None, None


def attention_packed(qkv, num_heads, key_padding_mask=None, causal=False, scale=None, dropout_p=0.0, seq=None):
    C = qkv.shape[-1] // 3
    if scale is None:
        scale = (C // num_heads) ** -0.5
    assert qkv.is_contiguous()
    if seq is not None:
        assert key_padding_mask is None and qkv.shape[0] == 1 and qkv.shape[1] == seq.rows
        return _AttnPackedFn.apply(qkv, None, seq.kv_len, num_heads, bool(causal), float(scale), *_drop_args(dropout_p), None, (seq.offsets, seq.longest))
    key_padding_mask, kv_len = _mask_and_len(key_padding_mask)
    pad_tiles = _pad_tiles(key_padding_mask) if (key_padding_mask is not None and qkv.requires_grad) else None
    return _AttnPackedFn.apply(qkv, key_padding_mask, kv_len, num_heads, bool(causal), float(scale), *_drop_args(dropout_p), pad_tiles)


class _StackedRowsFn(torch.autograd.Function):

    @staticmethod
    def forward(ctx, *ts):
        a = ts[0]
        ctx.rows, ctx.n = a.shape[0], len(ts)
        return torch.as_strided(a, (len(ts) * a.shape[0],) + tuple(a.shape[1:]), a.stride(), a.storage_offset())

    @staticmethod
    def backward(ctx, g):
        r = ctx.rows
        return tuple(g[i * r:(i + 1) * r] for i in range(ctx.n))


def stacked_rows(*ts):
    a = ts[0]
    n = a.numel() * a.element_size()
    if (not _os.environ.get("CST_NO_QKV_VIEW") and all(t.shape == a.shape and t.is_contiguous() for t in ts)
            and all(ts[i].data_ptr() + n == ts[i + 1].data_ptr() for i in range(len(ts) - 1))
            and a.untyped_storage().data_ptr() == ts[-1].untyped_storage().data_ptr()):
        K.STATS["qkv_view"] = K.STATS.get("qkv_view", 0) + 1
        out = _StackedRowsFn.apply(*ts)
        out._cst_parts = tuple(t.detach() for t in ts)
        out._cst_parts_params = tuple(ts)
        return out
    return torch.cat(ts, 0)


class PackedRows:

    def __init__(self, offsets, kv_len, rows, longest, B, T, host_lens=None):
        self.offsets, self.kv_len, self.rows, self.longest, self.B, self.T = offsets, kv_len, rows, longest, B, T
        self.host_lens = host_lens
        self.kept_host = None


def plan_packed_rows(padding_mask, margin):
    B, T = padding_mask.shape
    lens = (~padding_mask).sum(dim=1).to(torch.int32)
    n = torch.clamp(lens + (margin + 1), max=T)
    off = torch.zeros(B + 1, dtype=torch.int32, device=padding_mask.device)
    off[1:] = torch.cumsum(n, 0)
    host = torch.cat((off[-1:], n.max().view(1), lens)).tolist()
    plan = PackedRows(off.contiguous(), lens.contiguous(), int(host[0]), int(host[1]), B, T, [int(v) for v in host[2:]])
    plan.kept_host = [min(T, v + margin + 1) for v in plan.host_lens]
    return plan


def plan_from_lengths(lens_dev, host_lens, T):
    B = lens_dev.numel()
    n = torch.clamp(lens_dev.to(torch.int32), max=T)
    off = torch.zeros(B + 1, dtype=torch.int32, device=lens_dev.device)
    off[1:] = torch.cumsum(n, 0)
    hl = [min(int(v), T) for v in host_lens]
    return PackedRows(off.contiguous(), n.contiguous(), sum(hl), max(hl), B, T, hl)


class _PackRowsFn(torch.autograd.Function):

    @staticmethod
    def forward(ctx, x, seq):
        ctx.seq = seq
        return K.rows_pack(x.contiguous(), seq.offsets, seq.rows, tail_sum=False).unsqueeze(0)

    @staticmethod
    def backward(ctx, dy):
        s = ctx.seq
        dy2 = dy.reshape(s.rows, dy.shape[-1])
        return K.rows_unpack(dy2.contiguous(), s.offsets, s.B, s.T, tail_broadcast=False), None


class _UnpackRowsFn(torch.autograd.Function):

    @staticmethod
    def forward(ctx, y, seq, broadcast):
        ctx.seq, ctx.broadcast = seq, broadcast
        y2 = y.reshape(seq.rows, y.shape[-1])
        return K.rows_unpack(y2.contiguous(), seq.offsets, seq.B, seq.T, tail_broadcast=broadcast)

    @staticmethod
    def backward(ctx, dx):
        s = ctx.seq
        return K.rows_pack(dx.contiguous(), s.offsets, s.rows, tail_sum=ctx.broadcast).unsqueeze(0), None, None


def pack_rows(x, seq):
    return _PackRowsFn.apply(x, seq)


def unpack_rows(y, seq, broadcast=True):
    return _UnpackRowsFn.apply(y, seq, bool(broadcast))


def _conv0_args(wav, w, write_limit, grad_limit):
    C, _, k = w.shape
    if _os.environ.get("CST_NO_MLEN") or _os.environ.get("CST_GEMM_NO_KLIVE"):
        write_limit = grad_limit = None
    return wav.float().contiguous(), w.reshape(C, k).contiguous(), k, write_limit, grad_limit


class _Conv0Fn(torch.autograd.Function):
    @staticmethod
    def forward(ctx, wav, w, gamma, beta, stride, eps, write_limit, grad_limit):
        wav, w2, k, write_limit, grad_limit = _conv0_args(wav, w, write_limit, grad_limit)
        y, mean, rstd, gram = K.conv0_fwd(wav, w2, gamma, beta, k, stride, eps, frame_limit=write_limit)
        ctx.save_for_backward(wav, w2, gamma, beta, mean, rstd, gram)
        ctx.k, ctx.stride, ctx.grad_limit = k, stride, grad_limit
        return y

    @staticmethod
    def backward(ctx, dy):
        wav, w2, gamma, beta, mean, rstd, gram = ctx.saved_tensors
        dw, dg, db = K.conv0_bwd(dy.contiguous(), wav, w2, gamma, beta, mean, rstd, gram, ctx.k, ctx.stride, frame_limit=ctx.grad_limit)
        return None, dw.view(w2.shape[0], 1, ctx.k).to(w2.dtype), dg.to(gamma.dtype), db.to(gamma.dtype), None, None, None, None


def conv0_gn_gelu(wav, weight, gn_weight, gn_bias, stride, eps=1e-5, write_limit=None, grad_limit=None):
    return _Conv0Fn.apply(wav, weight, gn_weight, gn_bias, stride, eps, write_limit, grad_limit)


class _Conv0LnFn(torch.autograd.Function):
    @staticmethod
    def forward(ctx, wav, w, bias, gamma, beta, stride, eps, write_limit, grad_limit):
        wav, w2, k, write_limit, grad_limit = _conv0_args(wav, w, write_limit, grad_limit)
        y, mean, rstd = K.conv0_ln_fwd(wav, w2, bias, gamma, beta, k, stride, eps, frame_limit=write_limit)
        ctx.save_for_backward(wav, w2, bias, gamma, beta, mean, rstd)
        ctx.k, ctx.stride, ctx.grad_limit = k, stride, grad_limit
        return y

    @staticmethod
    def backward(ctx, dy):
        wav, w2, bias, gamma, beta, mean, rstd = ctx.saved_tensors
        dw, dbi, dg, db = K.conv0_ln_bwd(dy.contiguous(), wav, w2, bias, gamma, beta, mean, rstd, ctx.k, ctx.stride, frame_limit=ctx.grad_limit)
        return (None, dw.view(w2.shape[0], 1, ctx.k).to(w2.dtype), dbi.to(bias.dtype), dg.to(gamma.dtype), db.to(gamma.dtype),
# ... 538 lines not shown
```

chimera-st_amd/kernels.py:

```python
import ctypes
import os

import torch

from . import lib as L

_ws = {}
STATS = {}


def workspace(nbytes: int, device) -> torch.Tensor:
    key = (device.index, L.stream_ptr().value)
    t = _ws.get(key)
    if t is None or t.numel() < nbytes:
        t = torch.empty(max(nbytes, 1 << 20), dtype=torch.uint8, device=device)
        _ws[key] = t
    return t


class _Deferred:

    MAX_BYTES = 32 << 20

    def __init__(self):
# ... 183 lines not shown

def dw_colsum_is_fused(n_out, k_in, tokens, dtype):
    key = (n_out, k_in, tokens, dtype)
    r = _DW_FUSED.get(key)
    if r is None:
        d = L.GemmDesc()
        d.dtype = d.c_dtype = L.dtype_code(dtype)
        d.a_kmajor = d.b_kmajor = 0
        d.M, d.N, d.K = n_out, k_in, tokens
        d.batch0 = d.batch1 = 1
        d.split_k = -1
        d.colsum = 1
        r = _DW_FUSED[key] = bool(L.load().cst_gemm_colsum_is_fused(ctypes.byref(d)))
        if len(_DW_FUSED) > 4096:
            _DW_FUSED.clear()
    return r


def layernorm_fwd(x, res, gamma, beta, eps, want_sum=False):
    x = _2d(x)
    rows, cols = x.shape
    y = torch.empty_like(x)
    s = torch.empty_like(x) if (want_sum and res is not None) else None
    mean = torch.empty(rows, dtype=torch.float32, device=x.device)
    rstd = torch.empty(rows, dtype=torch.float32, device=x.device)
    L.check(L.load().cst_layernorm_fwd(L.ptr(x), L.ptr(res), L.ptr(gamma), L.ptr(beta), L.ptr(y), L.ptr(s), L.ptr(mean),
                                       L.ptr(rstd), rows, cols, eps, L.dtype_code(x.dtype), L.stream_ptr()), "cst_layernorm_fwd")
    return y, s, mean, rstd


_EPOCH = [0x3C6EF372]


def next_epoch():
    _EPOCH[0] = (_EPOCH[0] % 0xFFFFFFFE) + 1
    return _EPOCH[0]


def _two_stage(wbytes, outs, defer, launch):
    deferred = bool(defer) and DEFER.on > 0
    dev = outs[0].device
    ws = torch.empty(wbytes, dtype=torch.uint8, device=dev) if deferred else workspace(wbytes, dev)
    launch(ws, *[None if deferred else L.ptr(o) for o in outs])
    if deferred:
        n, cols = len(outs), outs[0].numel()
        for i, o in enumerate(outs):
            DEFER.push(ws.data_ptr() + 4 * cols * i, o, n * cols, cols, wbytes // (4 * n * cols), ws, order=1)


def layernorm_bwd(dy, s, gamma, mean, rstd, dres=None, grad_dtype=torch.float32, want_tiles=False, defer=False):
    dy, s = _2d(dy), _2d(s)
    rows, cols = s.shape
    lib = L.load()
    dx = torch.empty_like(s)
    dg = torch.empty(cols, dtype=grad_dtype, device=s.device)
    db = torch.empty(cols, dtype=grad_dtype, device=s.device)
    stamps, epoch = (torch.empty((rows + 63) // 64, dtype=torch.int32, device=s.device), next_epoch()) if want_tiles else (None, 0)

    def launch(ws, pg, pb):
        if want_tiles:
            L.check(lib.cst_layernorm_bwd_tiles(L.ptr(dy), L.ptr(s), L.ptr(gamma), L.ptr(mean), L.ptr(rstd), L.ptr(dres), L.ptr(dx), pg,
                                                pb, L.ptr(ws), rows, cols, L.dtype_code(s.dtype), L.dtype_code(grad_dtype),
                                                L.ptr(stamps), epoch, L.stream_ptr()), "cst_layernorm_bwd_tiles")
        else:
            L.check(lib.cst_layernorm_bwd(L.ptr(dy), L.ptr(s), L.ptr(gamma), L.ptr(mean), L.ptr(rstd), L.ptr(dres), L.ptr(dx), pg,
                                          pb, L.ptr(ws), rows, cols, L.dtype_code(s.dtype), L.dtype_code(grad_dtype), L.stream_ptr()),
                    "cst_layernorm_bwd")

    _two_stage(lib.cst_layernorm_bwd_workspace(rows, cols), (dg, db), defer, launch)
    return (dx, dg, db, (stamps, epoch)) if want_tiles else (dx, dg, db)


def _bhtd_strides(t, layout):
    assert t.stride(-1) == 1
    if layout == "bt":
        return t.stride(0), None, t.stride(1)
    return t.stride(1), None, t.stride(0)


def attn_desc(q, k, v, o, lse, H, D, kpm, causal, scale, layout_q="bt", layout_kv="bt", drop_p=0.0, drop_key=0, kv_len=None, seq=None):
    d = L.AttnDesc()
    d.dtype = L.dtype_code(q.dtype)
    if layout_q == "bt":
        B, Tq = q.shape[0], q.shape[1]
    else:
        Tq, B = q.shape[0], q.shape[1]
    Tk = k.shape[1] if layout_kv == "bt" else k.shape[0]
    if seq is not None:
        assert layout_q == "bt" and layout_kv == "bt" and B == 1 and kpm is None
        assert seq[0].dtype == torch.int32 and seq[0].is_contiguous()
        B, Tq, Tk = seq[0].numel() - 1, int(seq[1]), int(seq[1])
        d.seq_offsets = seq[0].data_ptr()
        STATS["attn_packed"] = STATS.get("attn_packed", 0) + 1
    else:
        d.seq_offsets = None
    d.B, d.H, d.Tq, d.Tk, d.D = B, H, Tq, Tk, D

    def st(t, lay):
        sb, _, stt = _bhtd_strides(t, lay)
        return sb, D, stt

    d.Q = q.data_ptr(); d.q_sb, d.q_sh, d.q_st = st(q, layout_q)
    d.K = k.data_ptr(); d.k_sb, d.k_sh, d.k_st = st(k, layout_kv)
    d.V = v.data_ptr(); d.v_sb, d.v_sh, d.v_st = st(v, layout_kv)
    d.O = o.data_ptr(); d.o_sb, d.o_sh, d.o_st = st(o, layout_q)
    d.lse = lse.data_ptr()
    if kpm is not None:
        assert kpm.dtype == torch.uint8 and kpm.stride(1) == 1 and kpm.shape == (B, Tk)
        d.key_padding_mask, d.kpm_stride = kpm.data_ptr(), kpm.stride(0)
        bits = kpm_bits(kpm)
        d.kpm_bits = bits.data_ptr()
        d._kpm_bits_owner = bits
    else:
        d.key_padding_mask, d.kpm_stride = None, 0
        d.kpm_bits = None
    d.bwd_ws = None
    d.causal, d.scale = int(causal), scale
    if q.dtype == torch.bfloat16 and D == 64 and not causal and not os.environ.get("CST_ATTN_GENERIC"):
        STATS["attn_fast"] = STATS.get("attn_fast", 0) + 1
    d.drop_p, d.drop_key = float(drop_p), int(drop_key) & 0xFFFFFFFF
    if kv_len is not None:
        assert (kpm is not None or seq is not None) and kv_len.dtype == torch.int32 and kv_len.numel() == B and kv_len.is_contiguous()
        d.kv_len = kv_len.data_ptr()
        STATS["attn_kv_len"] = STATS.get("attn_kv_len", 0) + 1
    else:
        d.kv_len = None
    return d


_KPM_BITS = []
_BIT_WEIGHTS = {}


def kpm_bits(kpm):
    key = (kpm.data_ptr(), tuple(kpm.shape), kpm._version)
    for ptr, shape, ver, _, bits in _KPM_BITS:
        if (ptr, shape, ver) == key:
            return bits
    B, Tk = kpm.shape
    nw = (Tk + 63) // 64
    m = kpm != 0
    if nw * 64 != Tk:
        m = torch.cat([m, torch.ones(B, nw * 64 - Tk, dtype=torch.bool, device=kpm.device)], 1)
    w = _BIT_WEIGHTS.get(kpm.device)
    if w is None:
        w = _BIT_WEIGHTS[kpm.device] = torch.ones(64, dtype=torch.int64, device=kpm.device) << torch.arange(64, dtype=torch.int64, device=kpm.device)
    bits = (m.view(B, nw, 64).to(torch.int64) * w).sum(-1).contiguous()
    _KPM_BITS.append(key + (kpm, bits))
    if len(_KPM_BITS) > 8:
        _KPM_BITS.pop(0)
    return bits


def attn_fwd(q, k, v, H, D, kpm, causal, scale, layout_q="bt", layout_kv="bt", drop_p=0.0, drop_key=0, kv_len=None):
    o = torch.empty_like(q)
    if layout_q == "bt":
        B, Tq = q.shape[0], q.shape[1]
    else:
        Tq, B = q.shape[0], q.shape[1]
    lse = torch.empty(B, H, Tq, dtype=torch.float32, device=q.device)
    d = attn_desc(q, k, v, o, lse, H, D, kpm, causal, scale, layout_q, layout_kv, drop_p, drop_key, kv_len)
    L.check(L.load().cst_attn_fwd(ctypes.byref(d), L.stream_ptr()), "cst_attn_fwd")
    return o, lse


def attn_fwd_desc(d):
    L.check(L.load().cst_attn_fwd(ctypes.byref(d), L.stream_ptr()), "cst_attn_fwd")


def attn_bwd_desc(d):
    L.check(L.load().cst_attn_bwd(ctypes.byref(d), L.stream_ptr()), "cst_attn_bwd")


def attn_bwd_fill(d, do, dq, dk, dv, delta, D, layout_q="bt", layout_kv="bt"):
    def st(t, lay):
        sb, _, stt = _bhtd_strides(t, lay)
        return sb, D, stt

    d.dO = do.data_ptr(); d.do_sb, d.do_sh, d.do_st = st(do, layout_q)
    d.dQ = dq.data_ptr(); d.dq_sb, d.dq_sh, d.dq_st = st(dq, layout_q)
    d.dK = dk.data_ptr(); d.dk_sb, d.dk_sh, d.dk_st = st(dk, layout_kv)
    d.dV = dv.data_ptr(); d.dv_sb, d.dv_sh, d.dv_st = st(dv, layout_kv)
    d.delta = delta.data_ptr()
    flags = torch.empty(int(d.B) * int(d.H) * ((int(d.Tq) + 63) // 64), dtype=torch.uint8, device=do.device)
    d.q_flags = flags.data_ptr()
    STATS["attn_q_flags"] = STATS.get("attn_q_flags", 0) + 1
    d._q_flags_owner = flags
    ws = torch.empty(int(L.load().cst_attn_bwd_workspace(ctypes.byref(d))) // 4, dtype=torch.float32, device=do.device)
    d.bwd_ws = ws.data_ptr()
    d._bwd_ws_owner = ws


def attn_bwd(do, q, k, v, o, lse, H, D, kpm, causal, scale, layout_q="bt", layout_kv="bt", drop_p=0.0, drop_key=0, kv_len=None, seq=None,
             grads=None):
    dq, dk, dv = grads if grads is not None else (torch.empty_like(q), torch.empty_like(k), torch.empty_like(v))
    delta = torch.empty_like(lse)
    d = attn_desc(q, k, v, o, lse, H, D, kpm, causal, scale, layout_q, layout_kv, drop_p, drop_key, kv_len, seq)
    attn_bwd_fill(d, do, dq, dk, dv, delta, D, layout_q, layout_kv)
    attn_bwd_desc(d)
    return dq, dk, dv


def conv0_fwd(wav, w, gamma, beta, k, stride, eps=1e-5, frame_limit=None):
    assert wav.dtype == torch.float32 and wav.is_contiguous()
    B, S = wav.shape
    C = w.shape[0]
    Lo = (S - k) // stride + 1
    y = torch.empty(B, Lo, C, dtype=w.dtype, device=wav.device)
    mean = torch.empty(B, C, dtype=torch.float32, device=wav.device)
    rstd = torch.empty(B, C, dtype=torch.float32, device=wav.device)
    gram = torch.empty(B, k * k + k, dtype=torch.float32, device=wav.device)
    lib = L.load()
    ws = workspace(lib.cst_conv0_fwd_workspace(B, S, k, stride), wav.device)
    L.check(lib.cst_conv0_gn_gelu_fwd(L.ptr(wav), L.ptr(w), L.ptr(gamma), L.ptr(beta), L.ptr(y), L.ptr(mean), L.ptr(rstd),
                                      L.ptr(gram), L.ptr(ws), _lim(frame_limit, B), B, S, C, k, stride, eps, L.dtype_code(w.dtype),
                                      L.stream_ptr()), "cst_conv0_gn_gelu_fwd")
    return y, mean, rstd, gram


def _lim(frame_limit, B):
    if frame_limit is None:
        return None
    assert frame_limit.dtype == torch.int32 and frame_limit.numel() == B and frame_limit.is_contiguous()
    STATS["conv0_frame_limit"] = STATS.get("conv0_frame_limit", 0) + 1
    return L.ptr(frame_limit)


def conv0_bwd(dy, wav, w, gamma, beta, mean, rstd, gram, k, stride, frame_limit=None):
    B, S = wav.shape
    C = w.shape[0]
    lib = L.load()
    dw = torch.empty(C, k, dtype=torch.float32, device=wav.device)
    dg = torch.empty(C, dtype=torch.float32, device=wav.device)
    db = torch.empty(C, dtype=torch.float32, device=wav.device)
    ws = workspace(lib.cst_conv0_bwd_workspace(B, S, C, k, stride), wav.device)
    L.check(lib.cst_conv0_gn_gelu_bwd(L.ptr(dy), L.ptr(wav), L.ptr(w), L.ptr(gamma), L.ptr(beta), L.ptr(mean), L.ptr(rstd),
                                      L.ptr(gram), L.ptr(dw), L.ptr(dg), L.ptr(db), L.ptr(ws), _lim(frame_limit, B), B, S, C, k, stride,
                                      L.dtype_code(w.dtype), L.stream_ptr()), "cst_conv0_gn_gelu_bwd")
    return dw, dg, db


def conv0_ln_fwd(wav, w, bias, gamma, beta, k, stride, eps=1e-5, frame_limit=None):
    assert wav.dtype == torch.float32 and wav.is_contiguous()
    B, S = wav.shape
    C = w.shape[0]
    Lo = (S - k) // stride + 1
    y = torch.empty(B, Lo, C, dtype=w.dtype, device=wav.device)
    mean = torch.empty(B, Lo, dtype=torch.float32, device=wav.device)
    rstd = torch.empty(B, Lo, dtype=torch.float32, device=wav.device)
    L.check(L.load().cst_conv0_ln_gelu_fwd(L.ptr(wav), L.ptr(w), L.ptr(bias), L.ptr(gamma), L.ptr(beta), L.ptr(y), L.ptr(mean),
                                           L.ptr(rstd), _lim(frame_limit, B), B, S, C, k, stride, eps, L.dtype_code(w.dtype),
                                           L.stream_ptr()), "cst_conv0_ln_gelu_fwd")
    return y, mean, rstd


def conv0_ln_bwd(dy, wav, w, bias, gamma, beta, mean, rstd, k, stride, frame_limit=None):
    B, S = wav.shape
    C = w.shape[0]
    lib = L.load()
    dw = torch.empty(C, k, dtype=torch.float32, device=wav.device)
    dbi, dg, db = (torch.empty(C, dtype=torch.float32, device=wav.device) for _ in range(3))
    ws = workspace(lib.cst_conv0_ln_bwd_workspace(B, S, C, k, stride), wav.device)
    L.check(lib.cst_conv0_ln_gelu_bwd(L.ptr(dy), L.ptr(wav), L.ptr(w), L.ptr(bias), L.ptr(gamma), L.ptr(beta), L.ptr(mean),
                                      L.ptr(rstd), L.ptr(dw), L.ptr(dbi), L.ptr(dg), L.ptr(db), L.ptr(ws), _lim(frame_limit, B), B, S,
                                      C, k, stride, L.dtype_code(w.dtype), L.stream_ptr()), "cst_conv0_ln_gelu_bwd")
    return dw, dbi, dg, db


def _row_lim(row_limit, B):
    if row_limit is None:
        return None
    assert row_limit.dtype == torch.int32 and row_limit.numel() == B and row_limit.is_contiguous()
    return L.ptr(row_limit)


def ln_gelu_fwd(u, gamma, beta, eps=1e-5, row_limit=None):
    assert u.dim() == 3 and u.is_contiguous()
    B, Lr, C = u.shape
    y = torch.empty_like(u)
    mean = torch.empty(B, Lr, dtype=torch.float32, device=u.device)
    rstd = torch.empty(B, Lr, dtype=torch.float32, device=u.device)
    L.check(L.load().cst_ln_gelu_fwd(L.ptr(u), L.ptr(gamma), L.ptr(beta), L.ptr(y), L.ptr(mean), L.ptr(rstd), _row_lim(row_limit, B),
                                     B, Lr, C, eps, L.dtype_code(u.dtype), L.stream_ptr()), "cst_ln_gelu_fwd")
    return y, mean, rstd


def ln_gelu_bwd(dy, u, gamma, beta, mean, rstd, row_limit=None, want_colsum=False, padded=False):
    assert dy.is_contiguous() and u.is_contiguous()
    B, Lr, C = u.shape
    lib = L.load()
    if padded:
        full = torch.empty(B, Lr + 2, C, dtype=u.dtype, device=u.device)
        full[:, 0].zero_()
        full[:, Lr + 1].zero_()
        du = full[:, 1:1 + Lr]
    else:
        du = torch.empty_like(u)
    dg, db = (torch.empty(C, dtype=torch.float32, device=u.device) for _ in range(2))
    dc = torch.empty(C, dtype=torch.float32, device=u.device) if want_colsum else None
    ws = workspace(lib.cst_ln_gelu_bwd_workspace(B * Lr, C), u.device)
    L.check(lib.cst_ln_gelu_bwd(L.ptr(dy), L.ptr(u), L.ptr(gamma), L.ptr(beta), L.ptr(mean), L.ptr(rstd), L.ptr(du), du.stride(0),
                                L.ptr(dg), L.ptr(db), L.ptr(dc), L.ptr(ws), _row_lim(row_limit, B), B, Lr, C, L.dtype_code(u.dtype),
                                L.stream_ptr()), "cst_ln_gelu_bwd")
    return du, dg, db, dc


def glu_fwd(z):
    z = _2d(z)
    rows, C2 = z.shape
    y = torch.empty(rows, C2 // 2, dtype=z.dtype, device=z.device)
    L.check(L.load().cst_glu_fwd(L.ptr(z), L.ptr(y), rows, C2 // 2, L.dtype_code(z.dtype), L.stream_ptr()), "cst_glu_fwd")
    return y


def glu_bwd(dy, z):
    dy, z = _2d(dy), _2d(z)
    rows, C2 = z.shape
    dz = torch.empty_like(z)
    L.check(L.load().cst_glu_bwd(L.ptr(dy), L.ptr(z), L.ptr(dz), rows, C2 // 2, L.dtype_code(z.dtype), L.stream_ptr()), "cst_glu_bwd")
    return dz


def act_bwd(dy, z, act):
    assert dy.is_contiguous() and z.is_contiguous()
    dx = torch.empty_like(z)
    L.check(L.load().cst_act_bwd(L.ptr(dy), L.ptr(z), L.ptr(dx), z.numel(), act, L.dtype_code(z.dtype), L.stream_ptr()), "cst_act_bwd")
    return dx


def posconv_fwd(x, wg, bias, groups, m_len=None):
    B, T, C = x.shape
    k = wg.shape[2]
    assert x.is_contiguous() and wg.is_contiguous() and x.dtype == torch.bfloat16 and wg.dtype == x.dtype
    y = torch.empty_like(x)
    z = torch.empty_like(x)
    L.check(L.load().cst_posconv_fwd(L.ptr(x), L.ptr(wg), L.ptr(bias) if bias is not None else None, L.ptr(y), L.ptr(z),
                                     _per_batch(m_len, B, "gemm_m_len"), B, T, C, groups, k, L.stream_ptr()), "cst_posconv_fwd")
    return y, z


def posconv_dx(dz, wflip, dy, groups, m_len=None):
    B, T, C = dz.shape
    k = wflip.shape[2]
    assert dz.is_contiguous() and dy.is_contiguous() and wflip.is_contiguous() and dz.dtype == torch.bfloat16
    dx = torch.empty_like(dz)
    L.check(L.load().cst_posconv_dx(L.ptr(dz), L.ptr(wflip), L.ptr(dy), L.ptr(dx), _per_batch(m_len, B, "gemm_m_len"),
                                    B, T, C, groups, k, L.stream_ptr()), "cst_posconv_dx")
    return dx


def posconv_dw(dz, x, groups, k, db=None, k_live=None):
# ... 510 lines not shown
```

chimera-st_amd/lib.py:

```python
import ctypes
import os

import torch

_HERE = os.path.dirname(os.path.abspath(__file__))
LIB_PATH = os.path.join(_HERE, "libcst_hip.so")
ABI_VERSION = 13

F32, BF16 = 0, 1
ACT_NONE, ACT_RELU, ACT_GELU = 0, 1, 2
BIAS_NONE, BIAS_COL, BIAS_ROW = 0, 1, 2
K_GEMM, K_ATTN_FWD, K_ATTN_BWD, K_LAYERNORM, K_CONV0, K_ELEMENTWISE, K_LOSS, K_OPTIM = range(8)
KERNEL_CLASSES = ["gemm", "attn_fwd", "attn_bwd", "layernorm", "conv0", "elementwise", "loss", "optim"]

c_i64, c_int, c_f, c_p = ctypes.c_int64, ctypes.c_int, ctypes.c_float, ctypes.c_void_p


class GemmDesc(ctypes.Structure):
    _fields_ = [
        ("dtype", c_int), ("c_dtype", c_int), ("a_kmajor", c_int), ("b_kmajor", c_int),
        ("M", c_i64), ("N", c_i64), ("K", c_i64),
        ("A", c_p), ("lda", c_i64), ("a_seg", c_i64), ("a_seg_stride", c_i64),
        ("B", c_p), ("ldb", c_i64), ("b_seg", c_i64), ("b_seg_stride", c_i64),
        ("C", c_p), ("ldc", c_i64),
        ("bias", c_p), ("bias_mode", c_int), ("sbias0", c_i64), ("sbias1", c_i64),
        ("act", c_int),
        ("aux_out", c_p), ("ld_aux_out", c_i64),
        ("dact", c_int),
        ("aux_in", c_p), ("ld_aux_in", c_i64),
        ("resid", c_p), ("ld_resid", c_i64),
        ("alpha", c_f),
        ("drop_p", c_f), ("drop_key", ctypes.c_uint32),
        ("batch0", c_i64), ("batch1", c_i64),
        ("sa0", c_i64), ("sa1", c_i64), ("sb0", c_i64), ("sb1", c_i64), ("sc0", c_i64), ("sc1", c_i64),
        ("split_k", c_int),
        ("workspace", c_p), ("workspace_bytes", c_i64),
        ("k_live", c_p), ("k_epoch", ctypes.c_uint32),
        ("m_live", c_p), ("m_epoch", ctypes.c_uint32),
        ("k_len", c_p),
        ("m_len", c_p),
        ("colsum", c_p),
        ("defer_reduce", c_int),
    ]


class ReduceItem(ctypes.Structure):
    _fields_ = [("src", c_p), ("dst", c_p), ("stride", c_i64), ("L", c_i64), ("P", ctypes.c_int32), ("dst_dtype", ctypes.c_int32),
                ("block0", ctypes.c_int32), ("order", ctypes.c_int32)]


class AttnDesc(ctypes.Structure):
    _fields_ = [
        ("dtype", c_int),
        ("B", c_i64), ("H", c_i64), ("Tq", c_i64), ("Tk", c_i64), ("D", c_i64),
        ("Q", c_p), ("q_sb", c_i64), ("q_sh", c_i64), ("q_st", c_i64),
        ("K", c_p), ("k_sb", c_i64), ("k_sh", c_i64), ("k_st", c_i64),
        ("V", c_p), ("v_sb", c_i64), ("v_sh", c_i64), ("v_st", c_i64),
        ("O", c_p), ("o_sb", c_i64), ("o_sh", c_i64), ("o_st", c_i64),
        ("lse", c_p),
        ("key_padding_mask", c_p), ("kpm_stride", c_i64),
        ("causal", c_int), ("scale", c_f),
        ("drop_p", c_f), ("drop_key", ctypes.c_uint32),
        ("dO", c_p), ("do_sb", c_i64), ("do_sh", c_i64), ("do_st", c_i64),
        ("dQ", c_p), ("dq_sb", c_i64), ("dq_sh", c_i64), ("dq_st", c_i64),
        ("dK", c_p), ("dk_sb", c_i64), ("dk_sh", c_i64), ("dk_st", c_i64),
        ("dV", c_p), ("dv_sb", c_i64), ("dv_sh", c_i64), ("dv_st", c_i64),
        ("delta", c_p),
        ("kv_len", c_p),
        ("q_flags", c_p),
        ("seq_offsets", c_p),
        ("kpm_bits", c_p),
        ("bwd_ws", c_p),
    ]


class BeamDesc(ctypes.Structure):
    _fields_ = [
        ("dtype", c_int),
        ("bsz", c_i64), ("beam", c_i64), ("vocab", c_i64), ("max_len", c_i64),
        ("pad", c_i64), ("unk", c_i64), ("eos", c_i64), ("min_len", c_i64),
        ("unk_penalty", c_f), ("len_penalty", c_f), ("temperature", c_f),
        ("normalize_scores", c_int),
        ("logits", c_p), ("ld_logits", c_i64),
        ("step", c_p),
        ("tokens", c_p), ("scores", c_p), ("anc", c_p),
        ("cands_to_ignore", c_p), ("finished", c_p), ("nfinal", c_p), ("num_remaining", c_p),
        ("fin_tokens", c_p), ("fin_pos", c_p), ("fin_score", c_p), ("fin_len", c_p),
        ("workspace", c_p),
        ("members", c_i64), ("logits_n", c_p * 7), ("lprobs_out", c_p),
        ("no_repeat_ngram", c_i64), ("prefix_tokens", c_p), ("prefix_len", c_i64),
        ("sampling", c_i64), ("sample_topk", c_i64), ("sample_topp", c_f), ("sample_key", c_p),
        ("diverse_groups", c_i64), ("diverse_strength", c_f), ("diverse_siblings", c_i64), ("sibling_rate", c_f),
        ("fin_anc", c_p),
    ]


class LmFusionDesc(ctypes.Structure):
    _fields_ = [("lm_logits", c_p), ("lm_weight", c_f), ("lprobs_out", c_p)]


class LexDesc(ctypes.Structure):
    _fields_ = [("representation", c_i64), ("constraints", c_p), ("width", c_i64), ("workspace", c_p)]


LEX_TBL_W, LEX_SW, LEX_NEXT_MAX, LEX_WIDTH_MAX = 136, 44, 16, 65


def lex_states(workspace, bsz, beam):
    words = workspace.view(torch.int32)
    return words[bsz * LEX_TBL_W:bsz * LEX_TBL_W + 2 * bsz * beam * LEX_SW].view(2, bsz * beam, LEX_SW)


class FbankDesc(ctypes.Structure):
    _fields_ = [
        ("B", c_i64), ("S", c_i64), ("T", c_i64),
        ("wave", c_p), ("n_samples", c_p), ("out", c_p), ("n_frames", c_p),
        ("utterance_cmvn", c_int), ("norm_means", c_int), ("norm_vars", c_int),
        ("global_mean", c_p), ("global_std", c_p),
        ("global_first", c_int),
        ("specaugment", c_int),
        ("n_fmask", c_int), ("n_tmask", c_int),
        ("fmask", c_p), ("tmask", c_p),
        ("mask_mean", c_int), ("mask_value", c_f),
        ("workspace", c_p), ("workspace_bytes", c_i64),
    ]


SYMBOLS = [
    ("cst_last_error", ctypes.c_char_p, []),
    ("cst_version", c_int, []),
    ("cst_device_arch_ok", c_int, []),
    ("cst_prof_enable", None, [c_int]),
    ("cst_prof_query", c_i64, [c_int, ctypes.POINTER(ctypes.c_double), ctypes.POINTER(ctypes.c_double), ctypes.POINTER(ctypes.c_double)]),
    ("cst_layernorm_fwd", c_int, [c_p, c_p, c_p, c_p, c_p, c_p, c_p, c_p, c_i64, c_i64, c_f, c_int, c_p]),
    ("cst_layernorm_bwd_workspace", c_i64, [c_i64, c_i64]),
    ("cst_layernorm_bwd", c_int, [c_p, c_p, c_p, c_p, c_p, c_p, c_p, c_p, c_p, c_p, c_i64, c_i64, c_int, c_int, c_p]),
    ("cst_layernorm_bwd_tiles", c_int, [c_p, c_p, c_p, c_p, c_p, c_p, c_p, c_p, c_p, c_p, c_i64, c_i64, c_int, c_int, c_p, ctypes.c_uint32, c_p]),
    ("cst_gemm_workspace", c_i64, [ctypes.POINTER(GemmDesc)]),
    ("cst_gemm_colsum_is_fused", c_int, [ctypes.POINTER(GemmDesc)]),
    ("cst_gemm_splits", c_int, [ctypes.POINTER(GemmDesc)]),
    ("cst_gemm_route", c_int, [ctypes.POINTER(GemmDesc), ctypes.c_char_p, c_i64]),
    ("cst_reduce_multi", c_int, [ctypes.POINTER(ReduceItem), c_int, c_p]),
    ("cst_gemm", c_int, [ctypes.POINTER(GemmDesc), c_p]),
    ("cst_posconv_fwd", c_int, [c_p, c_p, c_p, c_p, c_p, c_p, c_i64, c_i64, c_i64, c_i64, c_i64, c_p]),
    ("cst_posconv_dx", c_int, [c_p, c_p, c_p, c_p, c_p, c_i64, c_i64, c_i64, c_i64, c_i64, c_p]),
    ("cst_posconv_dw", c_int, [c_p, c_p, c_p, c_p, c_p, ctypes.c_uint32, c_i64, c_i64, c_i64, c_i64, c_i64, c_p]),
    ("cst_prof_dump", c_i64, [c_int, ctypes.c_char_p, c_i64]),
    ("cst_gemm_reserve_cus", c_int, [c_int]),
    ("cst_transpose2d", c_int, [c_p, c_p, c_i64, c_i64, c_int, c_p]),
    ("cst_transpose2d_multi", c_int, [c_p, c_int, c_i64, c_int, c_p]),
    ("cst_weight_norm_workspace", c_i64, [c_i64, c_i64]),
    ("cst_weight_norm_fwd", c_int, [c_p, c_p, c_p, c_p, c_p, c_i64, c_i64, c_int, c_p]),
    ("cst_weight_norm_bwd", c_int, [c_p, c_p, c_p, c_p, c_p, c_p, c_p, c_i64, c_i64, c_int, c_p]),
    ("cst_attn_bwd_workspace", c_i64, [ctypes.POINTER(AttnDesc)]),
    ("cst_attn_fwd", c_int, [ctypes.POINTER(AttnDesc), c_p]),
    ("cst_attn_bwd", c_int, [ctypes.POINTER(AttnDesc), c_p]),
    ("cst_conv0_fwd_workspace", c_i64, [c_i64, c_i64, c_int, c_int]),
    ("cst_conv0_gn_gelu_fwd", c_int, [c_p, c_p, c_p, c_p, c_p, c_p, c_p, c_p, c_p, c_p, c_i64, c_i64, c_i64, c_int, c_int, c_f, c_int, c_p]),
    ("cst_conv0_bwd_workspace", c_i64, [c_i64, c_i64, c_i64, c_int, c_int]),
    ("cst_conv0_gn_gelu_bwd", c_int, [c_p, c_p, c_p, c_p, c_p, c_p, c_p, c_p, c_p, c_p, c_p, c_p, c_p, c_i64, c_i64, c_i64, c_int, c_int, c_int, c_p]),
    ("cst_conv0_ln_gelu_fwd", c_int, [c_p, c_p, c_p, c_p, c_p, c_p, c_p, c_p, c_p, c_i64, c_i64, c_i64, c_int, c_int, c_f, c_int, c_p]),
    ("cst_conv0_ln_bwd_workspace", c_i64, [c_i64, c_i64, c_i64, c_int, c_int]),
    ("cst_conv0_ln_gelu_bwd", c_int, [c_p, c_p, c_p, c_p, c_p, c_p, c_p, c_p, c_p, c_p, c_p, c_p, c_p, c_p, c_i64, c_i64, c_i64, c_int, c_int, c_int, c_p]),
    ("cst_ln_gelu_fwd", c_int, [c_p, c_p, c_p, c_p, c_p, c_p, c_p, c_i64, c_i64, c_i64, c_f, c_int, c_p]),
    ("cst_ln_gelu_bwd_workspace", c_i64, [c_i64, c_i64]),
    ("cst_ln_gelu_bwd", c_int, [c_p, c_p, c_p, c_p, c_p, c_p, c_p, c_i64, c_p, c_p, c_p, c_p, c_p, c_i64, c_i64, c_i64, c_int, c_p]),
    ("cst_glu_fwd", c_int, [c_p, c_p, c_i64, c_i64, c_int, c_p]),
    ("cst_glu_bwd", c_int, [c_p, c_p, c_p, c_i64, c_i64, c_int, c_p]),
    ("cst_act_bwd", c_int, [c_p, c_p, c_p, c_i64, c_int, c_int, c_p]),
    ("cst_act_fwd", c_int, [c_p, c_p, c_i64, c_int, c_int, c_p]),
    ("cst_colsum", c_int, [c_p, c_i64, c_p, c_i64, c_i64, c_int, c_p]),
    ("cst_colsum_workspace", c_i64, [c_i64, c_i64]),
    ("cst_colsum_typed", c_int, [c_p, c_i64, c_p, c_p, c_i64, c_i64, c_int, c_int, c_p]),
    ("cst_colsum_typed_live", c_int, [c_p, c_i64, c_p, c_p, c_i64, c_i64, c_int, c_int, c_p, ctypes.c_uint32, c_p]),
    ("cst_col2im1d", c_int, [c_p, c_p, c_p, c_i64, c_i64, c_i64, c_i64, c_int, c_int, c_int, c_int, c_int, c_p]),
    ("cst_mask_rows", c_int, [c_p, c_p, c_p, c_i64, c_i64, c_int, c_p]),
    ("cst_dropout", c_int, [c_p, c_p, c_i64, c_f, ctypes.c_uint32, c_int, c_p]),
    ("cst_rows_pack", c_int, [c_p, c_p, c_p, c_i64, c_i64, c_i64, c_int, c_int, c_p]),
    ("cst_rows_unpack", c_int, [c_p, c_p, c_p, c_i64, c_i64, c_i64, c_int, c_int, c_p]),
    ("cst_dec_linear", c_int, [c_p, c_p, c_p, c_p, c_p, c_i64, c_i64, c_i64, c_i64, c_i64, c_i64, c_int, c_p, c_i64, c_int, c_p]),
    ("cst_dec_ln_linear", c_int, [c_p, c_p, c_p, c_p, c_f, c_p, c_p, c_i64, c_i64, c_i64, c_i64, c_i64, c_i64, c_int, c_p, c_i64, c_int, c_p]),
    ("cst_dropout_colsum", c_int, [c_p, c_p, c_p, c_p, c_i64, c_i64, c_int, c_int, c_f, ctypes.c_uint32, c_p, ctypes.c_uint32, c_p]),
    ("cst_conv_row_limits", c_int, [c_p, c_p, c_p, c_int, c_i64, c_p, c_i64, c_int, c_p]),
    ("cst_dropout_scale", c_int, [c_p, c_p, c_i64, c_f, c_f, ctypes.c_uint32, c_int, c_p]),
    ("cst_embed_pos_fwd", c_int, [c_p, c_p, c_p, c_p, c_p, c_f, c_i64, c_p, c_i64, c_i64, c_i64, c_i64, c_i64, c_f, ctypes.c_uint32, c_int, c_p]),
    ("cst_embed_bwd", c_int, [c_p, c_p, c_p, c_f, c_i64, c_i64, c_i64, c_i64, c_f, ctypes.c_uint32, c_int, c_int, c_p]),
    ("cst_ls_ce_fwd", c_int, [c_p, c_p, c_p, c_p, c_p, c_i64, c_i64, c_f, c_i64, c_int, c_p]),
    ("cst_ls_ce_bwd", c_int, [c_p, c_p, c_p, c_p, c_p, c_i64, c_i64, c_f, c_i64, c_int, c_p]),
    ("cst_score_tokens", c_int, [c_p, ctypes.POINTER(c_p), c_i64, c_i64, c_p, c_i64, c_p, c_p, c_p, c_i64, c_i64, c_i64, c_int, c_p]),
    ("cst_ctc_fwd", c_int, [c_p, c_i64, c_i64, c_p, c_i64, c_p, c_p, c_i64, c_int, c_p, c_p, c_p, c_p, c_p, c_p, c_i64, c_i64, c_i64, c_int, c_p]),
    ("cst_ctc_bwd", c_int, [c_p, c_i64, c_i64, c_p, c_i64, c_p, c_p, c_i64, c_int, c_p, c_p, c_p, c_p, c_p, c_p, c_i64, c_i64, c_i64, c_i64, c_i64,
                            c_int, c_p]),
    ("cst_ctc_greedy", c_int, [c_p, c_i64, c_i64, c_p, c_i64, c_p, c_p, c_p, c_i64, c_i64, c_i64, c_int, c_p]),
    ("cst_w2v_negatives", c_int, [ctypes.c_uint32, c_i64, c_i64, c_i64, c_i64, c_p, c_p]),
    ("cst_infonce_fwd", c_int, [c_p, c_p, c_p, c_f, c_p, c_p, c_p, c_p, c_p, c_p, c_p, c_p, c_i64, c_i64, c_i64, c_int, c_p]),
    ("cst_infonce_bwd_x", c_int, [c_p, c_p, c_p, c_f, c_p, c_p, c_p, c_p, c_p, c_p, c_i64, c_i64, c_i64, c_int, c_p]),
    ("cst_infonce_bwd_y", c_int, [c_p, c_p, c_p, c_p, c_p, c_p, c_p, c_p, c_i64, c_i64, c_i64, c_int, c_p]),
    ("cst_gumbel_vq_workspace", c_i64, [c_i64, c_i64, c_i64]),
    ("cst_gumbel_vq_fwd", c_int, [c_p, c_p, c_p, ctypes.c_uint32, c_int, c_p, c_p, c_p, c_p, c_p, c_p, c_p, c_i64, c_i64, c_i64, c_i64, c_int, c_p]),
    ("cst_gumbel_vq_bwd", c_int, [c_p, c_p, ctypes.c_uint32, c_f, c_p, c_p, c_p, c_p, c_p, c_i64, c_i64, c_i64, c_int, c_p]),
    ("cst_contrastive_fwd", c_int, [c_p, c_p, c_p, c_p, c_p, c_p, c_p, c_i64, c_i64, c_i64, c_f, c_int, c_p]),
    ("cst_contrastive_bwd", c_int, [c_p, c_p, c_p, c_p, c_p, c_p, c_p, c_p, c_i64, c_i64, c_i64, c_f, c_int, c_p]),
    ("cst_sumsq_workspace", c_i64, []),
    ("cst_sumsq", c_int, [c_p, c_i64, c_p, c_p, c_int, c_p]),
    ("cst_adam_step", c_int, [c_p, c_p, c_p, c_p, c_p, c_i64, c_f, c_f, c_f, c_f, c_f, c_i64, c_p, c_int, c_int, c_p]),
    ("cst_beam_workspace", c_i64, [c_i64, c_i64]),
    ("cst_beam_init", c_int, [ctypes.POINTER(BeamDesc), c_p]),
    ("cst_beam_step", c_int, [ctypes.POINTER(BeamDesc), c_p]),
    ("cst_beam_step_lm", c_int, [ctypes.POINTER(BeamDesc), ctypes.POINTER(LmFusionDesc), c_p]),
    ("cst_lex_workspace", c_i64, [c_i64, c_i64, c_i64]),
    ("cst_lex_init", c_int, [ctypes.POINTER(BeamDesc), ctypes.POINTER(LexDesc), c_p]),
    ("cst_beam_step_lex", c_int, [ctypes.POINTER(BeamDesc), ctypes.POINTER(LmFusionDesc), ctypes.POINTER(LexDesc), c_p]),
    ("cst_dec_embed", c_int, [c_p, c_p, c_p, c_p, c_f, c_i64, c_p, c_i64, c_i64, c_i64, c_i64, c_int, c_p]),
    ("cst_dec_self_attn", c_int, [c_p, c_p, c_p, c_p, c_p, c_p, c_i64, c_i64, c_i64, c_i64, c_f, c_int, c_p]),
    ("cst_batch_by_size", c_i64, [c_p, c_i64, c_i64, c_i64, ctypes.c_int32, c_p]),
    ("cst_wav_info", c_int, [ctypes.c_char_p, c_p, c_p, c_p, c_p]),
    ("cst_wav_read_f32", c_i64, [ctypes.c_char_p, c_i64, c_i64, c_p, c_i64]),
    ("cst_edit_distance", c_i64, [c_p, c_i64, c_p, c_i64]),
    ("cst_dec_cross_attn", c_int, [c_p, c_p, c_p, c_p, c_p, c_p, c_i64, c_i64, c_i64, c_i64, c_i64, c_i64, c_f, c_int, c_p]),
    ("cst_fbank_workspace_bytes", c_i64, [c_i64, c_i64]),
    ("cst_fbank", c_int, [ctypes.POINTER(FbankDesc), c_p]),
    ("cst_dec_ln_q_cross_attn", c_int, [c_p, c_i64, c_p, c_p, c_p, c_f, c_p, c_p, c_p, c_p, c_p, c_i64, c_i64, c_i64, c_i64, c_i64, c_i64, c_f, c_int, c_p]),
    ("cst_attn_avg_probs", c_int, [c_p, c_i64, c_p, c_i64, c_i64, c_i64, c_p, c_p, c_i64, c_p, c_i64, c_i64, c_i64, c_i64, c_i64, c_i64, c_f, c_f,
                                   c_int, c_int, c_p]),
    ("cst_collate_pairs", c_int, [c_p, c_p, c_int, c_p, c_p, c_i64, c_p, c_i64, c_i64, c_i64, c_i64, c_i64, c_int, c_int, c_p, c_p]),
    ("cst_token_block_slices", c_i64, [c_p, c_i64, c_int, c_i64, c_i64, c_p, c_i64]),
    ("cst_token_block_index", c_int, [c_p, c_i64, c_p, c_i64, c_p]),
    ("cst_collate_blocks", c_int, [c_p, c_int, c_p, c_i64, c_p, c_i64, c_i64, c_i64, c_i64, c_p, c_p]),
]

_lib = None


def load():
    global _lib
    if _lib is not None:
        return _lib
    if not os.path.exists(LIB_PATH):
        raise RuntimeError(
            "chimera-st_amd: %s is missing — the HIP extension is the product path and there is no fallback. "
            "Build it with `python -c 'import __graft_entry__ as g; g.build()'` or `make -C chimera-st_amd/csrc`." % LIB_PATH)
    lib = ctypes.CDLL(LIB_PATH)
    for name, res, args in SYMBOLS:
        fn = getattr(lib, name)
        fn.restype = res
        fn.argtypes = args
    built = lib.cst_version()
    if built != ABI_VERSION:
        raise RuntimeError("chimera-st_amd: %s was built for ABI version %d, this package binds version %d (include/cst.h "
                           "CST_ABI_VERSION) — rebuild it with `make -C chimera-st_amd/csrc`." % (LIB_PATH, built, ABI_VERSION))
    _lib = lib
    return lib


def check(rc, what=""):
    if rc != 0:
        msg = load().cst_last_error()
        raise RuntimeError("libcst_hip %s failed (%d): %s" % (what, rc, msg.decode() if msg else "?"))


def dtype_code(t: torch.dtype) -> int:
    if t == torch.float32:
        return F32
    if t == torch.bfloat16:
        return BF16
    raise TypeError("chimera-st_amd kernels compute in float32 or bfloat16 storage, got %s" % t)


_DEV_INDEX = None


def stream_ptr():
    global _DEV_INDEX
    if _DEV_INDEX is None:
        _DEV_INDEX = torch.cuda.current_device()
    return ctypes.c_void_p(torch._C._cuda_getCurrentRawStream(_DEV_INDEX))


def ptr(t):
    if t is None:
        return None
    if not t.is_cuda:
        raise RuntimeError("chimera-st_amd: tensor is not on the GPU — the HIP path has no CPU fallback")
    return ctypes.c_void_p(t.data_ptr())


def prof_enable(on: bool):
    load().cst_prof_enable(1 if on else 0)


def prof_query():
    lib = load()
    out = {}
    for i, name in enumerate(KERNEL_CLASSES):
        ms, fl, by = ctypes.c_double(), ctypes.c_double(), ctypes.c_double()
        n = lib.cst_prof_query(i, ctypes.byref(ms), ctypes.byref(fl), ctypes.byref(by))
        out[name] = dict(launches=int(n), ms=ms.value, flops=fl.value, bytes=by.value)
    return out


def prof_dump(cls):
    lib = load()
    n = lib.cst_prof_dump(cls, None, 0)
    buf = ctypes.create_string_buffer(int(n) + 16)
    lib.cst_prof_dump(cls, buf, len(buf))
    out = []
    for line in buf.value.decode().splitlines():
# ... 4 lines not shown
```

include/cst.h:

```cpp
#ifndef CST_H
#define CST_H

#include <stdint.h>

#ifdef __cplusplus
extern "C" {
#endif

#define CST_ABI_VERSION 13

typedef enum { CST_F32 = 0, CST_BF16 = 1 } cst_dtype;

typedef enum {
  CST_OK = 0,
  CST_ERR_BAD_ARG = -1,
  CST_ERR_LAUNCH = -2,
  CST_ERR_WORKSPACE = -3,
  CST_ERR_UNSUPPORTED = -4
} cst_status;

typedef void* cst_stream;

const char* cst_last_error(void);
int cst_version(void);
int cst_device_arch_ok(void);

typedef enum {
  CST_K_GEMM = 0, CST_K_ATTN_FWD, CST_K_ATTN_BWD, CST_K_LAYERNORM, CST_K_CONV0, CST_K_ELEMENTWISE,
  CST_K_LOSS, CST_K_OPTIM, CST_K_NUM
} cst_kernel_class;
void cst_prof_enable(int on);
int64_t cst_prof_query(int kernel_class, double* total_ms, double* flops, double* bytes);
int64_t cst_prof_dump(int kernel_class, char* buf, int64_t cap);

int cst_layernorm_fwd(const void* x, const void* res, const void* gamma, const void* beta,
                      void* y, void* sum_out, float* mean, float* rstd,
                      int64_t rows, int64_t cols, float eps, int dtype, cst_stream stream);
int64_t cst_layernorm_bwd_workspace(int64_t rows, int64_t cols);
int cst_layernorm_bwd(const void* dy, const void* s, const void* gamma, const float* mean,
                      const float* rstd, const void* dres, void* dx, void* dgamma, void* dbeta,
                      void* workspace, int64_t rows, int64_t cols, int dtype, int grad_dtype, cst_stream stream);
int cst_layernorm_bwd_tiles(const void* dy, const void* s, const void* gamma, const float* mean,
                            const float* rstd, const void* dres, void* dx, void* dgamma, void* dbeta,
                            void* workspace, int64_t rows, int64_t cols, int dtype, int grad_dtype,
                            uint32_t* tile_live, uint32_t epoch, cst_stream stream);

typedef enum { CST_ACT_NONE = 0, CST_ACT_RELU = 1, CST_ACT_GELU = 2 } cst_act;
typedef enum { CST_BIAS_NONE = 0, CST_BIAS_COL = 1, CST_BIAS_ROW = 2 } cst_bias_mode;

typedef struct {
  int dtype;
  int c_dtype;
  int a_kmajor, b_kmajor;
  int64_t M, N, K;
  const void* A; int64_t lda, a_seg, a_seg_stride;
  const void* B; int64_t ldb, b_seg, b_seg_stride;
  void* C; int64_t ldc;
  const void* bias; int bias_mode;
  int64_t sbias0, sbias1;
  int act;
  void* aux_out; int64_t ld_aux_out;
  int dact;
  const void* aux_in; int64_t ld_aux_in;
  const void* resid; int64_t ld_resid;
  float alpha;
  float drop_p; uint32_t drop_key;
  int64_t batch0, batch1;
  int64_t sa0, sa1, sb0, sb1, sc0, sc1;
  int split_k;
  void* workspace; int64_t workspace_bytes;
  const uint32_t* k_live; uint32_t k_epoch;
  const uint32_t* m_live; uint32_t m_epoch;
  const int32_t* k_len;
  const int32_t* m_len;
  void* colsum;
  int defer_reduce;
} cst_gemm_desc;

int64_t cst_gemm_workspace(const cst_gemm_desc* d);
int cst_gemm_colsum_is_fused(const cst_gemm_desc* d);
int cst_gemm_splits(const cst_gemm_desc* d);
int cst_gemm_route(const cst_gemm_desc* d, char* out, int64_t out_bytes);
int cst_gemm_reserve_cus(int n);
int cst_gemm(const cst_gemm_desc* d, cst_stream stream);

int cst_posconv_fwd(const void* x, const void* w, const void* bias, void* y, void* z, const int32_t* m_len, int64_t B, int64_t T,
                    int64_t C, int64_t groups, int64_t k, cst_stream stream);
int cst_posconv_dx(const void* dz, const void* wflip, const void* dy, void* dx, const int32_t* m_len, int64_t B, int64_t T,
                   int64_t C, int64_t groups, int64_t k, cst_stream stream);
int cst_posconv_dw(const void* dz, const void* x, void* dw, void* db, const uint32_t* k_live, uint32_t k_epoch, int64_t B,
                   int64_t T, int64_t C, int64_t groups, int64_t k, cst_stream stream);

typedef struct {
  int dtype;
  int64_t B, H, Tq, Tk, D;
  const void* Q; int64_t q_sb, q_sh, q_st;
  const void* K; int64_t k_sb, k_sh, k_st;
  const void* V; int64_t v_sb, v_sh, v_st;
  void* O; int64_t o_sb, o_sh, o_st;
  float* lse;
  const uint8_t* key_padding_mask; int64_t kpm_stride;
  int causal;
  float scale;
  float drop_p; uint32_t drop_key;
  const void* dO; int64_t do_sb, do_sh, do_st;
  void* dQ; int64_t dq_sb, dq_sh, dq_st;
  void* dK; int64_t dk_sb, dk_sh, dk_st;
  void* dV; int64_t dv_sb, dv_sh, dv_st;
  float* delta;
  const int32_t* kv_len;
  uint8_t* q_flags;
  const int32_t* seq_offsets;
  const uint64_t* kpm_bits;
  void* bwd_ws;
} cst_attn_desc;

int64_t cst_attn_bwd_workspace(const cst_attn_desc* d);
int cst_attn_fwd(const cst_attn_desc* d, cst_stream stream);
int cst_attn_bwd(const cst_attn_desc* d, cst_stream stream);

int cst_conv_row_limits(const int32_t* nz_last, const int32_t* k, const int32_t* stride, int L, int64_t S, int32_t* out, int64_t B,
                        int smax, cst_stream stream);
int64_t cst_conv0_fwd_workspace(int64_t B, int64_t S, int k, int stride);
int cst_conv0_gn_gelu_fwd(const float* wav, const void* w, const void* gamma, const void* beta,
                          void* y, float* mean, float* rstd, float* gram, float* workspace, const int32_t* frame_limit, int64_t B,
                          int64_t S, int64_t C, int k, int stride, float eps, int dtype, cst_stream stream);
int64_t cst_conv0_bwd_workspace(int64_t B, int64_t S, int64_t C, int k, int stride);
int cst_conv0_gn_gelu_bwd(const void* dy, const float* wav, const void* w, const void* gamma,
                          const void* beta, const float* mean, const float* rstd, const float* gram,
                          float* dw, float* dgamma, float* dbeta, float* workspace, const int32_t* frame_limit,
                          int64_t B, int64_t S, int64_t C, int k, int stride, int dtype,
                          cst_stream stream);

int cst_conv0_ln_gelu_fwd(const float* wav, const void* w, const void* bias, const void* gamma, const void* beta, void* y,
                          float* mean, float* rstd, const int32_t* frame_limit, int64_t B, int64_t S, int64_t C, int k,
                          int stride, float eps, int dtype, cst_stream stream);
int64_t cst_conv0_ln_bwd_workspace(int64_t B, int64_t S, int64_t C, int k, int stride);
int cst_conv0_ln_gelu_bwd(const void* dy, const float* wav, const void* w, const void* bias, const void* gamma, const void* beta,
                          const float* mean, const float* rstd, float* dw, float* dbias, float* dgamma, float* dbeta,
                          float* workspace, const int32_t* frame_limit, int64_t B, int64_t S, int64_t C, int k, int stride,
                          int dtype, cst_stream stream);
int cst_ln_gelu_fwd(const void* u, const void* gamma, const void* beta, void* y, float* mean, float* rstd,
                    const int32_t* row_limit, int64_t B, int64_t L, int64_t C, float eps, int dtype, cst_stream stream);
int64_t cst_ln_gelu_bwd_workspace(int64_t rows, int64_t C);
int cst_ln_gelu_bwd(const void* dy, const void* u, const void* gamma, const void* beta, const float* mean, const float* rstd,
                    void* du, int64_t du_batch_stride, float* dgamma, float* dbeta, float* dcolsum, float* workspace,
                    const int32_t* row_limit, int64_t B, int64_t L, int64_t C, int dtype, cst_stream stream);

int cst_glu_fwd(const void* z, void* y, int64_t rows, int64_t C, int dtype, cst_stream stream);
int cst_glu_bwd(const void* dy, const void* z, void* dz, int64_t rows, int64_t C, int dtype, cst_stream stream);
int cst_act_bwd(const void* dy, const void* z, void* dx, int64_t n, int act, int dtype, cst_stream stream);
int cst_act_fwd(const void* x, void* y, int64_t n, int act, int dtype, cst_stream stream);
int cst_colsum(const void* x, int64_t ldx, float* out, int64_t rows, int64_t cols, int dtype, cst_stream stream);
int cst_dropout_colsum(const void* x, void* xd, void* out, void* workspace, int64_t rows, int64_t cols, int dtype, int out_dtype,
                       float p, uint32_t key, const uint32_t* row_live, uint32_t epoch, cst_stream stream);
int64_t cst_colsum_workspace(int64_t rows, int64_t cols);
int cst_colsum_typed(const void* x, int64_t ldx, void* out, void* workspace, int64_t rows, int64_t cols, int dtype, int out_dtype,
                     cst_stream stream);
int cst_colsum_typed_live(const void* x, int64_t ldx, void* out, void* workspace, int64_t rows, int64_t cols, int dtype,
                          int out_dtype, const uint32_t* row_live, uint32_t epoch, cst_stream stream);
int cst_col2im1d(const void* dcol, const void* z, void* dx, int64_t B, int64_t Lin, int64_t Lout,
                 int64_t C, int k, int stride, int pad, int dact, int dtype, cst_stream stream);
int64_t cst_weight_norm_workspace(int64_t R, int64_t C);
int cst_weight_norm_fwd(const void* v, const void* g, void* w, float* norm, void* workspace, int64_t R, int64_t C, int dtype, cst_stream stream);
int cst_weight_norm_bwd(const void* v, const void* g, const void* dw, const float* norm, void* dv, void* dg, void* workspace, int64_t R,
                        int64_t C, int dtype, cst_stream stream);
int cst_transpose2d(const void* src, void* dst, int64_t R, int64_t C, int dtype, cst_stream stream);
typedef struct cst_transpose_item {
  const void* src; void* dst;
  int64_t R, C;
  int64_t tile0;
} cst_transpose_item;
int cst_transpose2d_multi(const cst_transpose_item* items_dev, int n, int64_t total_tiles, int dtype, cst_stream stream);
#define CST_REDUCE_MAX_ITEMS 64
typedef struct cst_reduce_item {
  const float* src; void* dst;
  int64_t stride, L;
  int32_t P, dst_dtype, block0, order;
} cst_reduce_item;
int cst_reduce_multi(const cst_reduce_item* items, int n, cst_stream stream);
int cst_mask_rows(const void* x, const uint8_t* mask, void* y, int64_t rows, int64_t cols, int dtype, cst_stream stream);

int cst_rows_pack(const void* src, const int32_t* seq_off, void* dst, int64_t B, int64_t T, int64_t C, int tail_sum, int dtype,
                  cst_stream stream);
int cst_rows_unpack(const void* src, const int32_t* seq_off, void* dst, int64_t B, int64_t T, int64_t C, int tail_broadcast, int dtype,
                    cst_stream stream);

int cst_dropout(const void* x, void* y, int64_t n, float p, uint32_t key, int dtype, cst_stream stream);
int cst_dropout_scale(const void* x, void* y, int64_t n, float alpha, float p, uint32_t key, int dtype, cst_stream stream);

int cst_embed_pos_fwd(const int64_t* tokens, const uint8_t* pad_mask, const void* embed, const void* x, const float* pos_table,
                      float scale, int64_t pad_idx, void* out, int64_t B, int64_t T, int64_t C, int64_t V, int64_t pos_rows,
                      float drop_p, uint32_t drop_key, int dtype, cst_stream stream);
int cst_embed_bwd(const void* dy, const int64_t* tokens, void* dE, float scale, int64_t pad_idx, int64_t n, int64_t C, int64_t V,
                  float drop_p, uint32_t drop_key, int dtype, int grad_dtype, cst_stream stream);

int cst_ls_ce_fwd(const void* logits, const int64_t* target, float* out2, float* lse, float* row_ws,
                  int64_t rows, int64_t V, float eps, int64_t pad_idx, int dtype, cst_stream stream);
int cst_ls_ce_bwd(const void* logits, const int64_t* target, const float* lse, const float* gscale,
                  void* dlogits, int64_t rows, int64_t V, float eps, int64_t pad_idx, int dtype,
                  cst_stream stream);

int cst_score_tokens(const void* logits, const void* const* logits_n, int64_t members, int64_t ld, const int64_t* target, int64_t pad,
                     float* pos, float* score, int32_t* len, int64_t B, int64_t T, int64_t V, int dtype, cst_stream stream);

int cst_ctc_fwd(const void* logits, int64_t stride_t, int64_t stride_b, const int64_t* targets, int64_t Lmax, const int64_t* target_len,
                const int64_t* input_len, int64_t blank, int zero_infinity, float* nll, float* loss, float* lse, float* emit, float* alpha,
                float* beta, int64_t T, int64_t B, int64_t V, int dtype, cst_stream stream);
int cst_ctc_bwd(const void* logits, int64_t stride_t, int64_t stride_b, const int64_t* targets, int64_t Lmax, const int64_t* target_len,
                const int64_t* input_len, int64_t blank, int zero_infinity, const float* nll, const float* lse, const float* alpha,
                const float* beta, const float* gscale, void* dlogits, int64_t dstride_t, int64_t dstride_b, int64_t T, int64_t B,
                int64_t V, int dtype, cst_stream stream);
int cst_ctc_greedy(const void* logits, int64_t stride_t, int64_t stride_b, const int64_t* input_len, int64_t blank, int32_t* argmax_ws,
                   int32_t* ids, int32_t* counts, int64_t T, int64_t B, int64_t V, int dtype, cst_stream stream);

int cst_w2v_negatives(uint32_t key, int64_t B, int64_t M, int64_t K, int64_t Kx, int32_t* out, cst_stream stream);
int cst_infonce_fwd(const void* x, const void* y, const int32_t* idx, float inv_temp, float* nll, float* loss, int32_t* counters,
                    float* lse, float* nx, float* ny, int32_t* flags, float* logits_dbg, int64_t N, int64_t KP, int64_t D, int dtype,
                    cst_stream stream);
int cst_infonce_bwd_x(const void* x, const void* y, const int32_t* idx, float inv_temp, const float* lse, const float* nx,
                      const float* ny, const float* gscale, void* dx, float* pairs, int64_t N, int64_t KP, int64_t D, int dtype,
                      cst_stream stream);
int cst_infonce_bwd_y(const void* x, const void* y, const int64_t* perm, const int32_t* offs, const float* pairs, const float* nx,
                      const float* ny, void* dy, int64_t N, int64_t KP, int64_t D, int dtype, cst_stream stream);

int64_t cst_gumbel_vq_workspace(int64_t N, int64_t G, int64_t V);
int cst_gumbel_vq_fwd(const void* logits, const void* vars, const float* noise, uint32_t key, int training, void* q, int32_t* idx,
                      void* onehot, float* avg_probs, float* stats, float* exph, void* workspace, int64_t N, int64_t G, int64_t V, int64_t d,
                      int dtype, cst_stream stream);
int cst_gumbel_vq_bwd(const void* logits, const float* noise, uint32_t key, float inv_tau, const void* gy, const float* avg_probs,
                      const float* exph, const float* dppl, void* dl, int64_t N, int64_t G, int64_t V, int dtype, cst_stream stream);

int cst_contrastive_fwd(const void* a, const void* t, float* loss, float* loss_rows, float* sim, float* na, float* nt,
                        int64_t B, int64_t M, int64_t C, float temp, int dtype, cst_stream stream);
int cst_contrastive_bwd(const void* a, const void* t, const float* sim, const float* na, const float* nt,
                        const float* gscale, void* da, void* dt, int64_t B, int64_t M, int64_t C, float temp,
                        int dtype, cst_stream stream);

int64_t cst_sumsq_workspace(void);
int cst_sumsq(const void* x, int64_t n, float* out, float* workspace, int dtype, cst_stream stream);
int cst_adam_step(float* master, float* exp_avg, float* exp_avg_sq, const void* grad, void* model_param,
                  int64_t n, float lr, float beta1, float beta2, float eps, float weight_decay,
                  int64_t step, const float* grad_scale, int grad_dtype, int param_dtype,
                  cst_stream stream);

typedef struct {
  int dtype;
  int64_t bsz, beam, vocab, max_len;
  int64_t pad, unk, eos, min_len;
  float unk_penalty, len_penalty, temperature;
  int normalize_scores;
  const void* logits; int64_t ld_logits;
  int32_t* step;
  int64_t* tokens; float* scores; int32_t* anc;
  uint8_t* cands_to_ignore; uint8_t* finished; int32_t* nfinal; int32_t* num_remaining;
  int64_t* fin_tokens; float* fin_pos; float* fin_score; int32_t* fin_len;
  void* workspace;
  int64_t members;
  const void* logits_n[7];
  float* lprobs_out;
  int64_t no_repeat_ngram;
  const int64_t* prefix_tokens;
  int64_t prefix_len;
  int64_t sampling;
  int64_t sample_topk;
  float sample_topp;
  const uint32_t* sample_key;
  int64_t diverse_groups;
// ... 86 lines not shown
```

Measured before the change: 528.0.

## Precompute per-key dropout signature table and DMA it into LDS

Adds a small kernel that precomputes per-key dropout hash signatures into a global table once per attention call. The forward and dQ kernels then stream these signatures into LDS alongside the K/V tiles with buffer-to-LDS loads, instead of computing them on the fly each tile. This also lets them use a cheaper s_barrier instead of __syncthreads. The table is saved from forward and reused in backward. It only activates when dropout is on and the tile count is above a threshold, and it costs an extra launch and some global memory.

```diff
diff --git a/chimera-st_amd/csrc/attention.hip b/chimera-st_amd/csrc/attention.hip
--- a/chimera-st_amd/csrc/attention.hip
+++ b/chimera-st_amd/csrc/attention.hip
@@ -25,6 +25,7 @@
   uint8_t* q_flags;
   const int32_t* seq_off;
   const unsigned long long* kpm_bits; int64_t kpm_bits_stride;
+  const void* key_sigs;
 };
 
 struct SeqView { int64_t row0; int tq, tk; };
@@ -636,6 +637,8 @@
   p.seq_off = d->seq_offsets;
   p.kpm_bits = (const unsigned long long*)d->kpm_bits;
   p.kpm_bits_stride = (d->Tk + 63) / 64;
+  CST_REQUIRE((uintptr_t)d->key_sigs % 16 == 0, "cst_attn: key_sigs must be 16-byte aligned");
+  p.key_sigs = d->drop_p > 0.0f ? d->key_sigs : nullptr;
   if (p.seq_off) {
     CST_REQUIRE(d->Tq == d->Tk && d->key_padding_mask == nullptr, "cst_attn: packed sequences are self-attention (Tq == Tk = longest segment) without a key padding mask (kv_len gives the keys per sequence)");
     CST_REQUIRE(d->q_st == d->k_st && d->q_st == d->v_st, "cst_attn: packed Q/K/V must share one row stride");
@@ -656,6 +659,11 @@
 }
 void attn_set_lds(const void* fn) {
   (void)hipFuncSetAttribute(fn, hipFuncAttributeMaxDynamicSharedMemorySize, 96 * 1024);
+}
+
+void fa_key_sigs_launch(const AttnParams& p, int64_t Tk, hipStream_t s) {
+  const int nwords = (int)(cst_ceil_div(Tk, 64) * 64 * 8);
+  hipLaunchKernelGGL(fa_key_sigs_kernel, dim3((unsigned)cst_ceil_div(nwords, 256)), dim3(256), 0, s, (uint32_t*)const_cast<void*>(p.key_sigs), p.drop_key, nwords);
 }
 
 double attn_flops(const cst_attn_desc* d, double gemms) {
@@ -687,8 +695,11 @@
   if (attn_fast_ok(d)) {
     CstProfScope prof(CST_K_ATTN_FWD, s, attn_flops(d, 2.0), 0.0);
     const unsigned nblk = fa_grid(d->Tq, d->B, d->H);
-    const size_t lds = FA_NSLOT * FA_SLOT + 8 * (size_t)cst_ceil_div(d->Tk, 64) + (p.drop_thr ? 4096 : 0);
-    if (p.drop_thr) hipLaunchKernelGGL((fa_fwd_kernel<true>), dim3(nblk), dim3(256), lds, s, p);
+    const size_t lds = FA_NSLOT * FA_SLOT + (size_t)fa_kbits_bytes((int)cst_ceil_div(d->Tk, 64)) + (p.drop_thr ? 4096 : 0);
+    if (p.key_sigs) {
+      fa_key_sigs_launch(p, d->Tk, s);
+      hipLaunchKernelGGL((fa_fwd_kernel<true, true>), dim3(nblk), dim3(256), lds, s, p);
+    } else if (p.drop_thr) hipLaunchKernelGGL((fa_fwd_kernel<true>), dim3(nblk), dim3(256), lds, s, p);
     else hipLaunchKernelGGL((fa_fwd_kernel<false>), dim3(nblk), dim3(256), lds, s, p);
     return cst_check_launch("cst_attn_fwd");
   }
@@ -718,6 +729,8 @@
   if (!d) return 0;
   return (int64_t)d->B * d->H * cst_ceil_div(d->Tq, 64) * 64 * (int64_t)(2 * sizeof(float) + 32);
 }
+
+extern "C" int64_t cst_attn_key_sigs_bytes(int64_t Tk) { return Tk > 0 ? cst_ceil_div(Tk, 64) * 64 * 32 : 0; }
 
 extern "C" int cst_attn_bwd(const cst_attn_desc* d, cst_stream stream) {
   AttnParams p;
@@ -731,8 +744,12 @@
     static const bool delta_pass = getenv("CST_ATTN_DELTA_PASS") != nullptr;
     if (delta_pass) hipLaunchKernelGGL(fa_delta_kernel, dim3((unsigned)(Tq64 / 64), (unsigned)d->H, (unsigned)d->B), dim3(64), 0, s, p, ws, Tq64);
     const unsigned nq = fa_grid(d->Tq, d->B, d->H), nk = fa_grid(d->Tk, d->B, d->H);
-    const size_t lds_q = FA_NSLOT * FA_SLOT + 8 * (size_t)cst_ceil_div(d->Tk, 64) + (p.drop_thr ? 4096 : 0) + 16, lds_k = FA_NSLOT * (FA_SLOT + FA_STATS);
-    if (p.drop_thr) {
+    const size_t lds_q = FA_NSLOT * FA_SLOT + (size_t)fa_kbits_bytes((int)cst_ceil_div(d->Tk, 64)) + (p.drop_thr ? 4096 : 0) + 16, lds_k = FA_NSLOT * (FA_SLOT + FA_STATS);
+    if (p.key_sigs) {
+      if (!d->key_sigs_ready) fa_key_sigs_launch(p, d->Tk, s);
+      hipLaunchKernelGGL((fa_dq_kernel<true, true>), dim3(nq), dim3(256), lds_q, s, p, ws, Tq64);
+      hipLaunchKernelGGL((fa_dkv_kernel<true>), dim3(nk), dim3(256), lds_k, s, p, (const float*)ws, Tq64);
+    } else if (p.drop_thr) {
       hipLaunchKernelGGL((fa_dq_kernel<true>), dim3(nq), dim3(256), lds_q, s, p, ws, Tq64);
       hipLaunchKernelGGL((fa_dkv_kernel<true>), dim3(nk), dim3(256), lds_k, s, p, (const float*)ws, Tq64);
     } else {
diff --git a/chimera-st_amd/csrc/attention_fast.inc b/chimera-st_amd/csrc/attention_fast.inc
--- a/chimera-st_amd/csrc/attention_fast.inc
+++ b/chimera-st_amd/csrc/attention_fast.inc
@@ -100,6 +100,25 @@
   v.y = KEYS ? cst_asig_key(key, key2, r, w + 1) : cst_asig_row(key, key2, r, w + 1);
   *reinterpret_cast<uint2*>(dst + (tid >> 2) * 32 + (tid & 3) * 8) = v;
 }
+__device__ __forceinline__ unsigned fa_sig_lane(int wave, int lane) { return (unsigned)((wave & 1) * 1024 + lane * 16); }
+__device__ __forceinline__ void fa_dma_sigs(const fa_i32x4& rsG, unsigned lds, unsigned sv, int j, int wave) {
+  if (wave >= 2) fa_dma16(rsG, lds + (unsigned)(wave & 1) * 1024u, sv + (unsigned)j * 2048u);
+}
+__device__ __forceinline__ void fa_dma_tile5(const fa_i32x4& rsG, unsigned lds_sig, unsigned sv, const fa_i32x4& rsA, const fa_i32x4& rsB, unsigned lds,
+                                             unsigned a0, unsigned a1, unsigned b0, unsigned b1) {
+  unsigned keep;
+  asm volatile("s_mov_b32 %0, m0\n\ts_mov_b32 m0, %8\n\ts_nop 0\n\tbuffer_load_dwordx4 %9, %10, 0 offen lds\n\t"
+               "s_mov_b32 m0, %1\n\ts_nop 0\n\tbuffer_load_dwordx4 %2, %6, 0 offen lds\n\t"
+               "s_add_i32 m0, %1, 0x400\n\ts_nop 0\n\tbuffer_load_dwordx4 %3, %6, 0 offen lds\n\t"
+               "s_add_i32 m0, %1, 0x2000\n\ts_nop 0\n\tbuffer_load_dwordx4 %4, %7, 0 offen lds\n\t"
+               "s_add_i32 m0, %1, 0x2400\n\ts_nop 0\n\tbuffer_load_dwordx4 %5, %7, 0 offen lds\n\ts_mov_b32 m0, %0"
+               : "=&s"(keep) : "s"(lds), "v"(a0), "v"(a1), "v"(b0), "v"(b1), "s"(rsA), "s"(rsB), "s"(lds_sig), "v"(sv), "s"(rsG) : "memory");
+}
+__global__ __launch_bounds__(256) void fa_key_sigs_kernel(uint32_t* tab, uint32_t key, int nwords) {
+  const int i = (int)(blockIdx.x * 256u + threadIdx.x);
+  if (i < nwords) tab[i] = cst_asig_key(key, cst_drop_key2(key), (uint32_t)(i >> 3), i & 7);
+}
+__device__ __host__ __forceinline__ int fa_kbits_bytes(int ntmax) { return (8 * ntmax + 15) & ~15; }
 __device__ __forceinline__ cst_i32x16 fa_mask_block(const char* sigs, int blk, int lane, const cst_i32x4& own) {
   const cst_i32x4 a = *reinterpret_cast<const cst_i32x4*>(sigs + (blk * 32 + (lane & 31)) * 32 + 16 * (lane >> 5));
   return cst_asig_block(a, own);
@@ -173,8 +192,9 @@
 #define FA_STAMP(i) do { } while (0)
 #endif
 
-template <bool DROP>
+template <bool DROP, bool TAB = false>
 __global__ __launch_bounds__(256, 3) void fa_fwd_kernel(AttnParams p) {
+  static_assert(DROP || !TAB, "the signature table belongs to the dropout variant");
   extern __shared__ __attribute__((aligned(16))) char smem_raw[];
   const int tid = threadIdx.x, lane = tid & 63, hi = lane >> 5;
   const int wave = __builtin_amdgcn_readfirstlane(tid >> 6);
@@ -196,7 +216,7 @@
   const int ntiles = (kend + 63) >> 6;
   const int ntmax = (int)((p.Tk + 63) >> 6);
   unsigned long long* kbits = p.kpm_bits ? reinterpret_cast<unsigned long long*>(smem_raw + FA_NSLOT * FA_SLOT) : nullptr;
-  char* const sigs = smem_raw + FA_NSLOT * FA_SLOT + 8 * ntmax;
+  char* const sigs = smem_raw + FA_NSLOT * FA_SLOT + fa_kbits_bytes(ntmax);
   const unsigned lds0 = (unsigned)(uintptr_t)(__attribute__((address_space(3))) char*)smem_raw;
   const fa_i32x4 rsK = fa_rsrc(Kg, kend > 0 ? (uint32_t)((kend - 1) * p.k_st * 2 + 128) : 0u);
   const fa_i32x4 rsV = fa_rsrc(Vg, kend > 0 ? (uint32_t)((kend - 1) * p.v_st * 2 + 128) : 0u);
@@ -208,6 +228,17 @@
     fa_dma_tile4(rsK, rsV, lds0 + slot * FA_SLOT + wave * 2048, vk[0] + (unsigned)j * stepK, vk[1] + (unsigned)j * stepK,
                  vv[0] + (unsigned)j * stepV, vv[1] + (unsigned)j * stepV);
   };
+  const unsigned lds_sigs = lds0 + FA_NSLOT * FA_SLOT + (unsigned)fa_kbits_bytes(ntmax);
+  const fa_i32x4 rsG = fa_rsrc(p.key_sigs, TAB ? (uint32_t)(ntmax * 2048) : 0u);
+  const unsigned sgv = fa_sig_lane(wave, lane);
+  auto dma_tile_sigs = [&](int j2, int slot) {
+    if (wave >= 2)
+      fa_dma_tile5(rsG, lds_sigs + (unsigned)((j2 - 1) & 1) * 2048u + (unsigned)(wave & 1) * 1024u, sgv + (unsigned)(j2 - 1) * 2048u, rsK, rsV,
+                   lds0 + slot * FA_SLOT + wave * 2048, vk[0] + (unsigned)j2 * stepK, vk[1] + (unsigned)j2 * stepK,
+                   vv[0] + (unsigned)j2 * stepV, vv[1] + (unsigned)j2 * stepV);
+    else dma_tile(j2, slot);
+  };
+  if (TAB && ntiles > 0) fa_dma_sigs(rsG, lds_sigs, sgv, 0, wave);
   if (ntiles > 0) dma_tile(0, 0);
   if (ntiles > 1) dma_tile(1, 1);
 
@@ -218,7 +249,7 @@
   cst_i32x4 bsig = {0, 0, 0, 0};
   if (DROP) {
     bsig = cst_asig_row_frag(p.drop_key, dkey2, (uint32_t)((b * p.H + h) * p.Tq + q), hi);
-    fa_stage_sigs<true>(sigs, p.drop_key, dkey2, 0u, tid);
+    if (!TAB) fa_stage_sigs<true>(sigs, p.drop_key, dkey2, 0u, tid);
   }
   if (kbits) for (int j = tid; j < ntiles; j += 256) kbits[j] = p.kpm_bits[b * p.kpm_bits_stride + j];
   const FaLanes L = fa_lanes(lane);
@@ -237,7 +268,8 @@
   auto tile = [&](int j, auto slot_c) {
     constexpr int SLOT = decltype(slot_c)::value;
     const bool ahead = j + 2 < ntiles;
-    if (ahead) dma_tile(j + 2, (SLOT + 2) % FA_NSLOT);
+    if (TAB) { if (ahead) dma_tile_sigs(j + 2, (SLOT + 2) % FA_NSLOT); else if (j + 1 < ntiles) fa_dma_sigs(rsG, lds_sigs + (unsigned)((j + 1) & 1) * 2048u, sgv, j + 1, wave); }
+    else if (ahead) dma_tile(j + 2, (SLOT + 2) % FA_NSLOT);
     const char* sK = smem_raw + SLOT * FA_SLOT;
     const char* sV = sK + FA_IMG;
     const unsigned long long mb = fa_tile_bits(kbits, j, kend);
@@ -294,7 +326,7 @@
 #pragma unroll
       for (int i = 0; i < 8; ++i) pk[ks][i] = fa_pack2(s[ks][2 * i], s[ks][2 * i + 1]);
     if (DROP) {
-      if (j + 1 < ntiles) fa_stage_sigs<true>(sigs + ((j + 1) & 1) * 2048, p.drop_key, dkey2, (uint32_t)(64 * (j + 1)), tid);
+      if (!TAB && j + 1 < ntiles) fa_stage_sigs<true>(sigs + ((j + 1) & 1) * 2048, p.drop_key, dkey2, (uint32_t)(64 * (j + 1)), tid);
 #pragma unroll
       for (int ks = 0; ks < 2; ++ks) {
         const cst_i32x16 dm = fa_mask_block(sigs + (j & 1) * 2048, ks, lane, bsig);
@@ -313,7 +345,7 @@
           o[dt] = FA_MFMA(fa_ld_tr(sV, L.ta[dt] + ks * 4096 + t * 2048, L.tb[dt] + ks * 4096 + t * 2048), fp, o[dt]);
       }
     if (ahead) fa_wait_vm<4>(); else fa_wait_vm<0>();
-    if (DROP) __syncthreads();
+    if (DROP && !TAB) __syncthreads();
     else __builtin_amdgcn_s_barrier();
   };
   for (int j = 0; j < ntiles; j += 3) {
@@ -380,8 +412,9 @@
   return cm;
 }
 
-template <bool DROP>
+template <bool DROP, bool TAB = false>
 __global__ __launch_bounds__(256, 2) void fa_dq_kernel(AttnParams p, float* ws, int64_t Tq64) {
+  static_assert(DROP || !TAB, "the signature table belongs to the dropout variant");
   extern __shared__ __attribute__((aligned(16))) char smem_raw[];
   const int tid = threadIdx.x, lane = tid & 63, hi = lane >> 5;
   const int wave = __builtin_amdgcn_readfirstlane(tid >> 6);
@@ -407,8 +440,8 @@
   const int ntiles = (kend + 63) >> 6;
   const int ntmax = (int)((p.Tk + 63) >> 6);
   unsigned long long* kbits = p.kpm_bits ? reinterpret_cast<unsigned long long*>(smem_raw + FA_NSLOT * FA_SLOT) : nullptr;
-  char* const sigs = smem_raw + FA_NSLOT * FA_SLOT + 8 * ntmax;
-  int* const sh_nz = reinterpret_cast<int*>(smem_raw + FA_NSLOT * FA_SLOT + 8 * ntmax + (DROP ? 4096 : 0));
+  char* const sigs = smem_raw + FA_NSLOT * FA_SLOT + fa_kbits_bytes(ntmax);
+  int* const sh_nz = reinterpret_cast<int*>(smem_raw + FA_NSLOT * FA_SLOT + fa_kbits_bytes(ntmax) + (DROP ? 4096 : 0));
   const unsigned lds0 = (unsigned)(uintptr_t)(__attribute__((address_space(3))) char*)smem_raw;
   const fa_i32x4 rsK = fa_rsrc(Kg, kend > 0 ? (uint32_t)((kend - 1) * p.k_st * 2 + 128) : 0u);
   const fa_i32x4 rsV = fa_rsrc(Vg, kend > 0 ? (uint32_t)((kend - 1) * p.v_st * 2 + 128) : 0u);
@@ -420,6 +453,17 @@
     fa_dma_tile4(rsK, rsV, lds0 + slot * FA_SLOT + wave * 2048, vk[0] + (unsigned)j * stepK, vk[1] + (unsigned)j * stepK,
                  vv[0] + (unsigned)j * stepV, vv[1] + (unsigned)j * stepV);
   };
+  const unsigned lds_sigs = lds0 + FA_NSLOT * FA_SLOT + (unsigned)fa_kbits_bytes(ntmax);
+  const fa_i32x4 rsG = fa_rsrc(p.key_sigs, TAB ? (uint32_t)(ntmax * 2048) : 0u);
+  const unsigned sgv = fa_sig_lane(wave, lane);
+  auto dma_tile_sigs = [&](int j2, int slot) {
+    if (wave >= 2)
+      fa_dma_tile5(rsG, lds_sigs + (unsigned)((j2 - 1) & 1) * 2048u + (unsigned)(wave & 1) * 1024u, sgv + (unsigned)(j2 - 1) * 2048u, rsK, rsV,
+                   lds0 + slot * FA_SLOT + wave * 2048, vk[0] + (unsigned)j2 * stepK, vk[1] + (unsigned)j2 * stepK,
+                   vv[0] + (unsigned)j2 * stepV, vv[1] + (unsigned)j2 * stepV);
+    else dma_tile(j2, slot);
+  };
+  if (TAB && ntiles > 0) fa_dma_sigs(rsG, lds_sigs, sgv, 0, wave);
   if (ntiles > 0) dma_tile(0, 0);
   if (ntiles > 1) dma_tile(1, 1);
 
@@ -465,7 +509,7 @@
   cst_i32x4 bsig = {0, 0, 0, 0};
   if (DROP) {
     bsig = cst_asig_row_frag(p.drop_key, dkey2, (uint32_t)((b * p.H + h) * p.Tq + q), hi);
-    fa_stage_sigs<true>(sigs, p.drop_key, dkey2, 0u, tid);
+    if (!TAB) fa_stage_sigs<true>(sigs, p.drop_key, dkey2, 0u, tid);
     if (q < Tq64) {
       cst_i32x4* sg = reinterpret_cast<cst_i32x4*>(reinterpret_cast<char*>(ws + (size_t)p.B * p.H * 2 * Tq64) + ((size_t)(b * p.H + h) * Tq64 + q) * 32 + 16 * hi);
       *sg = bsig;
@@ -495,12 +539,13 @@
   auto tile = [&](int j, auto slot_c) {
     constexpr int SLOT = decltype(slot_c)::value;
     const bool ahead = j + 2 < ntiles;
-    if (ahead) dma_tile(j + 2, (SLOT + 2) % FA_NSLOT);
+    if (TAB) { if (ahead) dma_tile_sigs(j + 2, (SLOT + 2) % FA_NSLOT); else if (j + 1 < ntiles) fa_dma_sigs(rsG, lds_sigs + (unsigned)((j + 1) & 1) * 2048u, sgv, j + 1, wave); }
+    else if (ahead) dma_tile(j + 2, (SLOT + 2) % FA_NSLOT);
     const char* sK = smem_raw + SLOT * FA_SLOT;
     const char* sV = sK + FA_IMG;
     const unsigned long long mb = fa_tile_bits(kbits, j, kend);
     const unsigned long long mbl = mb >> (4 * hi);
-    if (DROP && j + 1 < ntiles) fa_stage_sigs<true>(sigs + ((j + 1) & 1) * 2048, p.drop_key, dkey2, (uint32_t)(64 * (j + 1)), tid);
+    if (DROP && !TAB && j + 1 < ntiles) fa_stage_sigs<true>(sigs + ((j + 1) & 1) * 2048, p.drop_key, dkey2, (uint32_t)(64 * (j + 1)), tid);
 #pragma unroll
     for (int ks = 0; ks < 2; ++ks) {
       f32x16 s, dp;
@@ -529,7 +574,7 @@
       }
     }
     if (ahead) fa_wait_vm<4>(); else fa_wait_vm<0>();
-    if (DROP) __syncthreads();
+    if (DROP && !TAB) __syncthreads();
     else __builtin_amdgcn_s_barrier();
   };
   for (int j = 0; j < ntiles; j += 3) {
diff --git a/chimera-st_amd/functional.py b/chimera-st_amd/functional.py
--- a/chimera-st_amd/functional.py
+++ b/chimera-st_amd/functional.py
@@ -445,16 +445,17 @@
     @staticmethod
     def forward(ctx, q, k, v, kpm, kvl, H, causal, scale, layout_q, layout_kv, drop_p, drop_key):
         D = q.shape[-1] // H
-        o, lse = K.attn_fwd(q, k, v, H, D, kpm, causal, scale, layout_q, layout_kv, drop_p, drop_key, kvl)
-        ctx.save_for_backward(q, k, v, o, lse, kpm, kvl)
+        sigs = []
+        o, lse = K.attn_fwd(q, k, v, H, D, kpm, causal, scale, layout_q, layout_kv, drop_p, drop_key, kvl, key_sigs=sigs)
+        ctx.save_for_backward(q, k, v, o, lse, kpm, kvl, sigs[0])
         ctx.cfg = (H, D, causal, scale, layout_q, layout_kv, drop_p, drop_key)
         return o
 
     @staticmethod
     def backward(ctx, do):
-        q, k, v, o, lse, kpm, kvl = ctx.saved_tensors
+        q, k, v, o, lse, kpm, kvl, sigs = ctx.saved_tensors
         H, D, causal, scale, lq, lkv, drop_p, drop_key = ctx.cfg
-        dq, dk, dv = K.attn_bwd(_laid_out_like(do, o), q, k, v, o, lse, H, D, kpm, causal, scale, lq, lkv, drop_p, drop_key, kvl)
+        dq, dk, dv = K.attn_bwd(_laid_out_like(do, o), q, k, v, o, lse, H, D, kpm, causal, scale, lq, lkv, drop_p, drop_key, kvl, key_sigs=sigs)
         return dq, dk, dv, None, None, None, None, None, None, None, None, None
 
 
@@ -465,18 +466,19 @@
         C = kv.shape[-1] // 2
         D = C // H
         k, v = kv[..., :C], kv[..., C:]
-        o, lse = K.attn_fwd(q, k, v, H, D, kpm, False, scale, "bt", "bt", drop_p, drop_key, kvl)
-        ctx.save_for_backward(q, kv, o, lse, kpm, kvl)
+        sigs = []
+        o, lse = K.attn_fwd(q, k, v, H, D, kpm, False, scale, "bt", "bt", drop_p, drop_key, kvl, key_sigs=sigs)
+        ctx.save_for_backward(q, kv, o, lse, kpm, kvl, sigs[0])
         ctx.cfg = (H, D, C, scale, drop_p, drop_key)
         return o
 
     @staticmethod
     def backward(ctx, do):
-        q, kv, o, lse, kpm, kvl = ctx.saved_tensors
+        q, kv, o, lse, kpm, kvl, sigs = ctx.saved_tensors
         H, D, C, scale, drop_p, drop_key = ctx.cfg
         dq, dkv = torch.empty_like(q), torch.empty_like(kv)
         K.attn_bwd(_laid_out_like(do, o), q, kv[..., :C], kv[..., C:], o, lse, H, D, kpm, False, scale, "bt", "bt", drop_p, drop_key, kvl,
-                   grads=(dq, dkv[..., :C], dkv[..., C:]))
+                   grads=(dq, dkv[..., :C], dkv[..., C:]), key_sigs=sigs)
         return dq, dkv, None, None, None, None, None, None
 
 
@@ -527,14 +529,15 @@
         o = torch.empty(B, T, C, dtype=qkv.dtype, device=qkv.device)
         lse = torch.empty((seq[0].numel() - 1) if seq is not None else B, H, int(seq[1]) if seq is not None else T, dtype=torch.float32, device=qkv.device)
         d = K.attn_desc(q, k, v, o, lse, H, D, kpm, causal, scale, "bt", "bt", drop_p, drop_key, kvl, seq)
+        sigs = K.attn_key_sigs(d, qkv.device)
         K.attn_fwd_desc(d)
-        ctx.save_for_backward(qkv, o, lse, kpm, kvl, seq[0] if seq is not None else None)
+        ctx.save_for_backward(qkv, o, lse, kpm, kvl, seq[0] if seq is not None else None, sigs)
         ctx.cfg = (H, D, C, causal, scale, drop_p, drop_key, int(seq[1]) if seq is not None else None)
         return o
 
     @staticmethod
     def backward(ctx, do):
-        qkv, o, lse, kpm, kvl, seq_off = ctx.saved_tensors
+        qkv, o, lse, kpm, kvl, seq_off, sigs = ctx.saved_tensors
         H, D, C, causal, scale, drop_p, drop_key, seq_max = ctx.cfg
         seq = (seq_off, seq_max) if seq_off is not None else None
         live = _tiles_of(do, qkv.shape[0] * qkv.shape[1]) if ctx.pad_tiles is not None else None
@@ -542,7 +545,7 @@
             do = do.contiguous()
         dqkv = torch.empty_like(qkv)
         K.attn_bwd(do, qkv[..., :C], qkv[..., C:2 * C], qkv[..., 2 * C:], o, lse, H, D, kpm, causal, scale, "bt", "bt", drop_p, drop_key, kvl, seq,
-                   grads=(dqkv[..., :C], dqkv[..., C:2 * C], dqkv[..., 2 * C:]))
+                   grads=(dqkv[..., :C], dqkv[..., C:2 * C], dqkv[..., 2 * C:]), key_sigs=sigs)
         if live is not None:
             stamps = torch.where(ctx.pad_tiles, live[0], torch.full_like(live[0], live[1] if live[1] < 2 ** 31 else live[1] - 2 ** 32))
             dqkv = _with_tiles(dqkv, (stamps, live[1]))
diff --git a/chimera-st_amd/kernels.py b/chimera-st_amd/kernels.py
--- a/chimera-st_amd/kernels.py
+++ b/chimera-st_amd/kernels.py
@@ -359,7 +359,26 @@
     return bits
 
 
-def attn_fwd(q, k, v, H, D, kpm, causal, scale, layout_q="bt", layout_kv="bt", drop_p=0.0, drop_key=0, kv_len=None):
+KEY_SIGS_MIN_TILES = 16384
+
+
+def attn_key_sigs(d, device, table=None):
+    if not d.drop_p > 0.0:
+        return None
+    if table is None and int(d.B) * int(d.H) * ((int(d.Tq) + 127) // 128) * ((int(d.Tk) + 63) // 64) < KEY_SIGS_MIN_TILES:
+        return None
+    if table is None:
+        table = torch.empty(int(L.load().cst_attn_key_sigs_bytes(int(d.Tk))) // 4, dtype=torch.int32, device=device)
+        d.key_sigs_ready = 0
+    else:
+        assert table.dtype == torch.int32 and table.is_contiguous() and table.numel() * 4 == L.load().cst_attn_key_sigs_bytes(int(d.Tk))
+        d.key_sigs_ready = 1
+    d.key_sigs = table.data_ptr()
+    d._key_sigs_owner = table
+    return table
+
+
+def attn_fwd(q, k, v, H, D, kpm, causal, scale, layout_q="bt", layout_kv="bt", drop_p=0.0, drop_key=0, kv_len=None, key_sigs=None):
     o = torch.empty_like(q)
     if layout_q == "bt":
         B, Tq = q.shape[0], q.shape[1]
@@ -367,6 +386,10 @@
         Tq, B = q.shape[0], q.shape[1]
     lse = torch.empty(B, H, Tq, dtype=torch.float32, device=q.device)
     d = attn_desc(q, k, v, o, lse, H, D, kpm, causal, scale, layout_q, layout_kv, drop_p, drop_key, kv_len)
+    if key_sigs is not False:
+        table = attn_key_sigs(d, q.device)
+        if key_sigs is not None:
+            key_sigs.append(table)
     L.check(L.load().cst_attn_fwd(ctypes.byref(d), L.stream_ptr()), "cst_attn_fwd")
     return o, lse
 
@@ -399,11 +422,13 @@
 
 
 def attn_bwd(do, q, k, v, o, lse, H, D, kpm, causal, scale, layout_q="bt", layout_kv="bt", drop_p=0.0, drop_key=0, kv_len=None, seq=None,
-             grads=None):
+             grads=None, key_sigs=None):
     dq, dk, dv = grads if grads is not None else (torch.empty_like(q), torch.empty_like(k), torch.empty_like(v))
     delta = torch.empty_like(lse)
     d = attn_desc(q, k, v, o, lse, H, D, kpm, causal, scale, layout_q, layout_kv, drop_p, drop_key, kv_len, seq)
     attn_bwd_fill(d, do, dq, dk, dv, delta, D, layout_q, layout_kv)
+    if key_sigs is not False:
+        attn_key_sigs(d, do.device, key_sigs)
     attn_bwd_desc(d)
     return dq, dk, dv
 
diff --git a/chimera-st_amd/lib.py b/chimera-st_amd/lib.py
--- a/chimera-st_amd/lib.py
+++ b/chimera-st_amd/lib.py
@@ -71,6 +71,7 @@
         ("seq_offsets", c_p),
         ("kpm_bits", c_p),
         ("bwd_ws", c_p),
+        ("key_sigs", c_p), ("key_sigs_ready", c_int),
     ]
 
 
@@ -153,6 +154,7 @@
     ("cst_weight_norm_fwd", c_int, [c_p, c_p, c_p, c_p, c_p, c_i64, c_i64, c_int, c_p]),
     ("cst_weight_norm_bwd", c_int, [c_p, c_p, c_p, c_p, c_p, c_p, c_p, c_i64, c_i64, c_int, c_p]),
     ("cst_attn_bwd_workspace", c_i64, [ctypes.POINTER(AttnDesc)]),
+    ("cst_attn_key_sigs_bytes", c_i64, [c_i64]),
     ("cst_attn_fwd", c_int, [ctypes.POINTER(AttnDesc), c_p]),
     ("cst_attn_bwd", c_int, [ctypes.POINTER(AttnDesc), c_p]),
     ("cst_conv0_fwd_workspace", c_i64, [c_i64, c_i64, c_int, c_int]),
diff --git a/include/cst.h b/include/cst.h
--- a/include/cst.h
+++ b/include/cst.h
@@ -113,7 +113,11 @@
   const int32_t* seq_offsets;
   const uint64_t* kpm_bits;
   void* bwd_ws;
+  void* key_sigs;
+  int key_sigs_ready;
 } cst_attn_desc;
+
+int64_t cst_attn_key_sigs_bytes(int64_t Tk);
 
 int64_t cst_attn_bwd_workspace(const cst_attn_desc* d);
 int cst_attn_fwd(const cst_attn_desc* d, cst_stream stream);
```

Result: slower. 522.6 (-1.0%).
